# yamatokataoka/reinforcement-learning-replications

Hardware: AMD Instinct MI355X
Metric: env_steps_per_sec (higher is better)
Workload: dtype fp32; 1 GPU; model=PPO HalfCheetah-v4 (policy MLP [17,64,32,6] tanh, value [17,64,32,1]), global_batch=4000, seq_len=1000, parallelism=dp1, num_envs_per_gpu=200, env_residency=device, policy_grads_per_epoch=80

## Files before the change

rl_replicas_amd/algorithms/on_policy.py:

```python
from __future__ import annotations

import logging
from typing import Dict, List

import numpy as np
import torch
import torch.nn.functional as F
from torch import Tensor

from rl_replicas_amd import ops
from rl_replicas_amd.algorithms.base import AlgorithmBase
from rl_replicas_amd.experience import Experience
from rl_replicas_amd.policies import Policy
from rl_replicas_amd.samplers import Sampler
from rl_replicas_amd.value_function import ValueFunction

logger = logging.getLogger(__name__)


class OnPolicyAlgorithm(AlgorithmBase):
    def __init__(
        self,
        policy: Policy,
        value_function: ValueFunction,
        env,
        sampler: Sampler,
        gamma: float,
        gae_lambda: float,
        num_value_gradients: int,
    ) -> None:
        self.policy = policy
        self.value_function = value_function
        self.env = env
        self.sampler = sampler
        self.gamma = gamma
        self.gae_lambda = gae_lambda
        self.num_value_gradients = num_value_gradients

    def learn(
        self,
        num_epochs: int = 50,
        batch_size: int = 4000,
        model_saving_interval: int = 4000,
        output_dir: str = ".",
    ) -> None:
        import time as _time

        self._begin_learn(output_dir)
        for current_epoch in range(1, num_epochs + 1):
            t0 = _time.perf_counter()
            experience = self.sampler.sample(batch_size, self.policy)
            t1 = _time.perf_counter()

            self.current_total_steps += sum(experience.episode_lengths)
            self.current_total_episodes += sum(experience.episode_dones)

            self._record_sampling_metrics(
                current_epoch, experience.episode_returns, experience.episode_lengths
            )

            self.train(experience)

            self.metrics_manager.record_phase_ms("sample", (t1 - t0) * 1000.0)
            self.metrics_manager.record_phase_ms("train", (_time.perf_counter() - t1) * 1000.0)
            self.metrics_manager.dump_phases(self.current_total_steps)

            self._end_epoch(current_epoch, model_saving_interval, output_dir)
        self.metrics_manager.close()

    def _prepare_batch(self, experience: Experience) -> Dict[str, Tensor]:
        device = self.device
        flat = experience.to_flat_batch()
        if isinstance(flat["observations"], Tensor):
            obs = flat["observations"].to(device)
            actions = flat["actions"].to(device=device, dtype=torch.float32)
            rewards = flat["rewards"].to(device)
            last_obs = flat["last_observations"].to(device)
            return self._finish_batch(flat, obs, actions, rewards, last_obs, device)
        obs_np = flat["observations"]
        act_np = np.asarray(flat["actions"], dtype=np.float32)
        rew_np = flat["rewards"]
        last_np = flat["last_observations"]
        if device.type == "cuda":
            sizes = [a.size for a in (obs_np, act_np, rew_np, last_np)]
            total = int(sum(sizes))
            pinned = getattr(self, "_h2d_pinned", None)
            if pinned is None or pinned.numel() < total:
                pinned = torch.empty(total, dtype=torch.float32, pin_memory=True)
                self._h2d_pinned = pinned
                self._h2d_event = torch.cuda.Event()
            self._h2d_event.synchronize()
            host = pinned[:total].numpy()
            o = 0
            for a in (obs_np, act_np, rew_np, last_np):
                host[o : o + a.size] = a.reshape(-1)
                o += a.size
            dev_flat = pinned[:total].to(device, non_blocking=True)
            self._h2d_event.record()
            s0, s1, s2, s3 = np.cumsum(sizes)
            obs = dev_flat[:s0].view(obs_np.shape)
            actions = dev_flat[s0:s1].view(act_np.shape)
            rewards = dev_flat[s1:s2]
            last_obs = dev_flat[s2:s3].view(last_np.shape)
        else:
            obs = torch.as_tensor(obs_np, dtype=torch.float32, device=device)
            actions = torch.as_tensor(act_np, device=device)
            rewards = torch.as_tensor(rew_np, dtype=torch.float32, device=device)
            last_obs = torch.as_tensor(last_np, dtype=torch.float32, device=device)
        return self._finish_batch(flat, obs, actions, rewards, last_obs, device)

    def _finish_batch(self, flat, obs, actions, rewards, last_obs, device) -> Dict[str, Tensor]:
        offsets = torch.as_tensor(flat["episode_offsets"], device=device)
        dones = torch.as_tensor(flat["episode_dones"], device=device)

        with torch.no_grad():
            values_all = self.value_function(torch.cat([obs, last_obs], dim=0)).flatten()
        num_steps = obs.shape[0]
        values = values_all[:num_steps]
        last_values = values_all[num_steps:]

        advantages, returns = ops.gae_advantages_and_returns(
            rewards, values, last_values, offsets, dones, self.gamma, self.gae_lambda
        )
        obs, actions, advantages, returns = self._gather_global_batch(
            obs, actions, advantages, returns
        )
        advantages = self._normalize_advantages(advantages)
        return {
            "observations": obs,
            "actions": actions,
            "advantages": advantages.detach(),
            "discounted_returns": returns.detach(),
        }

    def _gather_global_batch(self, obs, actions, advantages, returns):
        return obs, actions, advantages, returns

    def _normalize_advantages(self, advantages: Tensor) -> Tensor:
        return ops.normalize(advantages)

    def train(self, experience: Experience) -> None:
        batch = self._prepare_batch(experience)
        obs = batch["observations"]
        actions = batch["actions"]
        advantages = batch["advantages"]
        returns = batch["discounted_returns"]

        joint = self._update_policy_and_value(obs, actions, advantages, returns)
        if joint is not None:
            policy_metrics, value_loss = joint
        else:
            policy_metrics = self._update_policy(obs, actions, advantages)
            value_loss = self._update_value_function(obs, returns)

        m = self.metrics_manager
        for tag, value in policy_metrics.items():
            m.record_scalar(tag, value, self.current_total_steps, tensorboard=True)
        m.record_scalar(
            "value_function/average_loss",
            value_loss,
            self.current_total_steps,
            tensorboard=True,
        )

    def _update_policy(self, obs: Tensor, actions: Tensor, advantages: Tensor) -> Dict[str, float]:
        raise NotImplementedError

    def _update_policy_and_value(self, obs: Tensor, actions: Tensor, advantages: Tensor,
                                 returns: Tensor):
        return None

    def _update_value_function(self, obs: Tensor, returns: Tensor) -> float:
        from rl_replicas_amd.ops import fused_onpolicy

        if fused_onpolicy.value_supported(self, obs):
            return fused_onpolicy.value_update(self, obs, returns, self.num_value_gradients)
        value_losses: List[float] = []
        for _ in range(self.num_value_gradients):
            value_losses.append(self.train_value_function(obs, returns).item())
        return float(np.mean(value_losses))

    def _policy_diagnostics(self, obs: Tensor, actions: Tensor) -> Dict[str, float]:
        with torch.no_grad():
            dist = self.policy(obs)
            log_probs = dist.log_prob(actions)
            entropies = dist.entropy()
        return {
            "policy/avarage_entropy": float(torch.mean(entropies)),
            "policy/log_prob_std": float(torch.std(log_probs)),
        }

    def train_value_function(self, observations: Tensor, discounted_returns: Tensor) -> Tensor:
        loss = self.compute_value_function_loss(observations, discounted_returns)
        self.value_function.optimizer.zero_grad()
        loss.backward()
        self._all_reduce_gradients(self.value_function)
        self.value_function.optimizer.step()
        return loss.detach()

    def compute_value_function_loss(self, observations: Tensor, discounted_returns: Tensor) -> Tensor:
        values = torch.squeeze(self.value_function(observations), -1)
        return F.mse_loss(values, discounted_returns)

    def _all_reduce_gradients(self, module) -> None:
        """DP hook: no-op single-process; the parallel wrapper overrides."""

    def _checkpoint_dict(self, epoch: int) -> Dict:
        return {
            "epoch": epoch,
            "total_steps": self.current_total_steps,
            "policy_state_dict": self.policy.network.state_dict(),
            "policy_optimizer_state_dict": self.policy.optimizer.state_dict(),
            "value_function_state_dict": self.value_function.network.state_dict(),
            "value_function_optimizer_state_dict": self.value_function.optimizer.state_dict(),
        }

    def _restore_from_checkpoint(self, ckpt: Dict) -> None:
        self.policy.network.load_state_dict(ckpt["policy_state_dict"])
        self.policy.optimizer.load_state_dict(ckpt["policy_optimizer_state_dict"])
        self.value_function.network.load_state_dict(ckpt["value_function_state_dict"])
        self.value_function.optimizer.load_state_dict(ckpt["value_function_optimizer_state_dict"])
```

rl_replicas_amd/algorithms/ppo.py:

```python
from __future__ import annotations

import copy
import logging
from typing import Dict

import torch
from torch import Tensor

from rl_replicas_amd.algorithms.on_policy import OnPolicyAlgorithm
from rl_replicas_amd.policies import Policy
from rl_replicas_amd.samplers import Sampler
from rl_replicas_amd.value_function import ValueFunction

logger = logging.getLogger(__name__)


class PPO(OnPolicyAlgorithm):
    def __init__(
        self,
        policy: Policy,
        value_function: ValueFunction,
        env,
        sampler: Sampler,
        gamma: float = 0.99,
        gae_lambda: float = 0.97,
        clip_range: float = 0.2,
        max_kl_divergence: float = 0.01,
        num_policy_gradients: int = 80,
        num_value_gradients: int = 80,
    ) -> None:
        super().__init__(policy, value_function, env, sampler, gamma, gae_lambda, num_value_gradients)
        self.clip_range = clip_range
        self.max_kl_divergence = max_kl_divergence
        self.num_policy_gradients = num_policy_gradients
        self.old_policy: Policy = copy.deepcopy(self.policy)

    def _update_policy(self, obs: Tensor, actions: Tensor, advantages: Tensor) -> Dict[str, float]:
        from rl_replicas_amd.ops import fused_onpolicy

        if fused_onpolicy.supported(self.policy, obs):
            return fused_onpolicy.ppo_update(self, obs, actions, advantages)
        diagnostics = self._policy_diagnostics(obs, actions)
        with torch.no_grad():
            loss_before = self.compute_policy_loss(obs, actions, advantages)

        with torch.no_grad():
            old_log_probs = self.old_policy(obs).log_prob(actions)

        approximate_kl = torch.zeros((), device=obs.device)
        for i in range(self.num_policy_gradients):
            self.train_policy(obs, actions, advantages, old_log_probs)
            with torch.no_grad():
                log_probs = self.policy(obs).log_prob(actions)
                approximate_kl = torch.mean(old_log_probs - log_probs)
            approximate_kl = self._reduce_scalar_mean(approximate_kl)
            if float(approximate_kl) > 1.5 * self.max_kl_divergence:
                logger.info(
                    "Early stopping at update %d due to reaching max KL divergence.", i
                )
                break

        self.old_policy.load_state_dict(self.policy.state_dict())

        return {
            "policy/loss": float(loss_before),
            **diagnostics,
            "policy/kl_divergence": float(approximate_kl),
        }

    def _update_policy_and_value(self, obs: Tensor, actions: Tensor, advantages: Tensor,
                                 returns: Tensor):
        from rl_replicas_amd.ops import fused_onpolicy

        if fused_onpolicy.ppo_twin_eligible(self, obs):
            return fused_onpolicy.ppo_value_twin_update(self, obs, actions, advantages, returns)
        return None

    def train_policy(self, obs: Tensor, actions: Tensor, advantages: Tensor, old_log_probs: Tensor) -> None:
        loss = self._clipped_loss(obs, actions, advantages, old_log_probs)
        self.policy.optimizer.zero_grad()
        loss.backward()
        self._all_reduce_gradients(self.policy)
        self.policy.optimizer.step()

    def _clipped_loss(self, obs: Tensor, actions: Tensor, advantages: Tensor, old_log_probs: Tensor) -> Tensor:
        log_probs = self.policy(obs).log_prob(actions)
        ratio = torch.exp(log_probs - old_log_probs)
        clipped_ratio = torch.clamp(ratio, 1.0 - self.clip_range, 1.0 + self.clip_range)
        return -torch.mean(torch.min(ratio * advantages, clipped_ratio * advantages))

    def compute_policy_loss(self, observations: Tensor, actions: Tensor, advantages: Tensor) -> Tensor:
        with torch.no_grad():
            old_log_probs = self.old_policy(observations).log_prob(actions)
        return self._clipped_loss(observations, actions, advantages, old_log_probs)

    def compute_approximate_kl_divergence(self, observations: Tensor, actions: Tensor) -> Tensor:
        with torch.no_grad():
            log_probs = self.policy(observations).log_prob(actions)
            old_log_probs = self.old_policy(observations).log_prob(actions)
        return torch.mean(old_log_probs - log_probs)
```

rl_replicas_amd/ops/fused_onpolicy.py:

```python
from __future__ import annotations

import gc
import logging
import math
import os
from typing import Dict, List, Optional

import numpy as np
import torch
from torch import Tensor

from rl_replicas_amd import ops
from rl_replicas_amd.ops.fused_mlp import _extract_layers
from rl_replicas_amd.policies import CategoricalPolicy, GaussianPolicy

logger = logging.getLogger(__name__)

MODE_VPG = 0
MODE_PPO = 1


def _policy_kind(policy) -> Optional[str]:
    if isinstance(policy, GaussianPolicy):
        return "gaussian"
# ... 356 lines not shown
                "policy/kl_divergence": float(self.kl_final[0]),
            }
        loss_before = None
        approximate_kl = 0.0
        for i in range(algo.num_policy_gradients):
            scalars = self.pre.replay()
            algo._all_reduce_gradients(policy)
            kl = self.post.replay()
            if loss_before is None:
                loss_before = float(scalars[0])
            approximate_kl = float(algo._reduce_scalar_mean(kl[0]))
            if approximate_kl > 1.5 * algo.max_kl_divergence:
                logger.info(
                    "Early stopping at update %d due to reaching max KL divergence.", i
                )
                break
        return {"policy/loss": loss_before, "policy/kl_divergence": approximate_kl}


def _value_iter_wide(algo, obs: Tensor, returns: Tensor, adam=None) -> Tensor:
    ext = ops._load_extension()
    vf = algo.value_function
    mlp = vf.network
    out, hidden, weights, biases, acts = _forward_saved(mlp, obs)
    dv, scalars = ext.value_mse_loss(out.view(-1), returns)
    if adam is not None:
        m, v, step0, hp, delta = adam
        ext.mlp_backward(dv.view(out.shape), obs, list(weights),
                         list(biases), list(hidden), out, acts,
                         ops.compute_bf16(), m, v, step0, *hp, delta)
        return scalars
    grads = ext.mlp_backward(dv.view(out.shape), obs, list(weights),
                             list(biases), list(hidden), out, acts,
                             ops.compute_bf16())
    _assign_grads(weights, biases, grads)
    return scalars


class _GraphedValueLoop:

    def __init__(self, algo, obs0: Tensor, returns0: Tensor, num_iters: int,
                 split: bool, mode: str = "narrow"):
        ext = ops._load_extension()
        vf = algo.value_function
        mlp = vf.network
        self.obs = obs0.clone()
        self.returns = returns0.clone()
        self.num_iters = num_iters
        self.split = split

        if mode == "wide":
            self._init_wide(algo, vf, num_iters, split)
            return

        def iter_pre():
            out, hidden, weights, biases, acts = _forward_saved(mlp, self.obs)
            grads = ext.value_mlp_backward(self.obs, list(weights), list(biases),
                                           list(hidden), out, acts, self.returns,
                                           ops.compute_bf16())
            _assign_grads(weights, biases, grads)
            return grads[-1]

        state = [p.data for p in vf.parameters()]
        state += _ensure_adam_state(vf.optimizer)
        if split:
            self.pre = _CapturedLoop(iter_pre, state)
            self.post = _CapturedLoop(lambda: vf.optimizer.step(), state)
        else:
            fb = int(ext.value_loss_partials_blocks(obs0.shape[0]))
            self.partials = torch.zeros(num_iters, fb, device=obs0.device)
            from rl_replicas_amd.ops.fused_adam import adam_arg_lists

            weights0, biases0, _ = _extract_layers(mlp)
            adam_m, adam_v, adam_step, hp = adam_arg_lists(
                vf.optimizer, weights0, biases0
            )

            fp32 = ops.compute_bf16() == 0 and _fwd_in_kernel_fits(weights0)
            dummy = torch.empty(0, device=obs0.device)

            def body():
                weights, biases, acts = _extract_layers(mlp)
                for i in range(num_iters):
                    if fp32:
                        ext.value_mlp_backward(
                            self.obs, list(weights), list(biases), [],
                            dummy, acts, self.returns, 0,
                            self.partials[i], adam_m, adam_v, adam_step,
                            *hp, float(i), True,
                        )
                    else:
                        out, hidden, _, _, _ = _forward_saved(mlp, self.obs)
                        ext.value_mlp_backward(
                            self.obs, list(weights), list(biases), list(hidden),
                            out, acts, self.returns, ops.compute_bf16(),
                            self.partials[i], adam_m, adam_v, adam_step,
                            *hp, float(i),
                        )
                vf.optimizer.bump_steps(float(num_iters))
                return ext.value_loss_finalize(self.partials, fb)

            self.loop = _CapturedLoop(body, state)

    def _init_wide(self, algo, vf, num_iters: int, split: bool) -> None:

        def iter_pre():
            return _value_iter_wide(algo, self.obs, self.returns)

        state = [p.data for p in vf.parameters()]
        state += _ensure_adam_state(vf.optimizer)
        if split:
            self.pre = _CapturedLoop(iter_pre, state)
            self.post = _CapturedLoop(lambda: vf.optimizer.step(), state)
        else:
            losses_buf = torch.zeros(num_iters, device=self.obs.device)
            from rl_replicas_amd.ops.fused_adam import adam_arg_lists

            weights0, biases0, _ = _extract_layers(vf.network)
            adam_m, adam_v, adam_step, hp = adam_arg_lists(
                vf.optimizer, weights0, biases0
            )

            def body():
                for i in range(num_iters):
                    losses_buf[i].copy_(
                        _value_iter_wide(
                            algo, self.obs, self.returns,
                            adam=(adam_m, adam_v, adam_step, hp, float(i)),
                        )[0]
                    )
                vf.optimizer.bump_steps(float(num_iters))
                return losses_buf

            self.loop = _CapturedLoop(body, state)

    def run(self, algo, obs, returns) -> float:
        self.obs.copy_(obs)
        self.returns.copy_(returns)
        if self.split:
            losses = []
            for _ in range(self.num_iters):
                losses.append(self.pre.replay().clone())
                algo._all_reduce_gradients(algo.value_function)
                self.post.replay()
            return float(torch.cat(losses).mean())
        losses = self.loop.replay()
        return float(losses.mean())


class _GraphedPPOTwin:

    def __init__(self, algo, obs0: Tensor, actions0: Tensor, adv0: Tensor,
                 old_logp0: Tensor, returns0: Tensor):
        from rl_replicas_amd.ops.fused_adam import adam_arg_lists

        ext = ops._load_extension()
        policy, vf = algo.policy, algo.value_function
        pmlp, vmlp = _mlp_of(policy), vf.network
        dev = obs0.device
        self.obs = obs0.clone()
        self.actions = actions0.clone()
        self.adv = adv0.clone()
        self.old_logp = old_logp0.clone()
        self.returns = returns0.clone()
        clip = float(algo.clip_range)
        thr = 1.5 * float(algo.max_kl_divergence)
        num_p = int(algo.num_policy_gradients)
        num_v = int(algo.num_value_gradients)
        assert 1 <= num_p <= num_v
        self.gate = torch.ones(1, device=dev)
        self.kl_final = torch.zeros(1, device=dev)
        self.loss0 = torch.zeros(1, device=dev)
        self.iters_done = torch.zeros(1, device=dev)
        scratch_loss = torch.zeros(1, device=dev)

        pw, pb, pacts = _extract_layers(pmlp)
        pm, pv, pstep, php = adam_arg_lists(policy.optimizer, pw, pb)
        state = [p.data for p in policy.parameters()]
        state += _ensure_adam_state(policy.optimizer)
        kind = _policy_kind(policy)
        self.kind = kind
        twin_iter, seed_args, ls_mv = _policy_iter_binding(
            ext, policy, kind, twin=True
        )

        vw, vb, vacts = _extract_layers(vmlp)
        vm, vv, vstep, vhp = adam_arg_lists(vf.optimizer, vw, vb)
        state += [p.data for p in vf.parameters()]
        state += _ensure_adam_state(vf.optimizer)
        fb = int(ext.value_loss_partials_blocks(obs0.shape[0]))
        self.partials = torch.zeros(num_v, fb, device=dev)
        dummy = torch.empty(0, device=dev)

        def body():
            self.gate.fill_(1.0)
            self.iters_done.zero_()
            for i in range(num_p):
                twin_iter(
                    self.obs, list(pw), list(pb), pacts, self.actions,
                    self.old_logp, self.adv, *seed_args, clip, pm,
                    pv, *ls_mv, pstep, *php, float(i), self.gate,
                    self.kl_final, self.iters_done, thr,
                    self.loss0 if i == 0 else scratch_loss, i == 0,
                    self.obs, list(vw), list(vb), vacts, self.returns,
                    self.partials[i], vm, vv, vstep, *vhp, float(i),
                )
            for i in range(num_p, num_v):
                ext.value_mlp_backward(
                    self.obs, list(vw), list(vb), [], dummy, vacts,
                    self.returns, 0, self.partials[i], vm, vv, vstep, *vhp,
                    float(i), True,
                )
            out = _forward_only(pmlp, self.obs)
            if kind == "gaussian":
                kl = ext.gaussian_kl(out, self.actions, policy.log_std.data,
                                     self.old_logp)
            else:
                kl = ext.categorical_kl(out, self.actions, self.old_logp)
            ext.ppo_gate_update_(self.gate, kl, self.kl_final,
                                 self.iters_done, thr)
            policy.optimizer.bump_steps_by(self.iters_done)
            vf.optimizer.bump_steps(float(num_v))
            return ext.value_loss_finalize(self.partials, fb)

        self.loop = _CapturedLoop(body, state)

    def run(self, algo, obs, actions, advantages, old_logp, returns):
        self.obs.copy_(obs)
        self.actions.copy_(actions.view(self.actions.shape))
        self.adv.copy_(advantages)
        self.old_logp.copy_(old_logp)
        self.returns.copy_(returns)
        losses = self.loop.replay()
        iters = int(self.iters_done)
        if iters < algo.num_policy_gradients:
            logger.info(
                "Early stopping at update %d due to reaching max KL divergence.",
                iters - 1,
            )
        return {
            "policy/loss": float(self.loss0[0]),
            "policy/kl_divergence": float(self.kl_final[0]),
        }, float(losses.mean())


def _get_cached_graph(algo, attr: str, key, builder):
    cached = getattr(algo, attr, None)
    if cached is not None and cached[0] == key:
        return cached[1]
    graph = builder()
    setattr(algo, attr, (key, graph))
    return graph


def _kernel_inputs(policy, obs: Tensor, actions: Tensor, advantages: Tensor):
    kind = _policy_kind(policy)
    obs = obs.contiguous()
    if kind == "gaussian":
        actions_k = actions.contiguous().view(obs.shape[0], -1)
    else:
        actions_k = actions.contiguous().view(-1)
    advantages = advantages.contiguous()
    diagnostics = _fast_diagnostics(policy, kind, obs, actions_k)
    return kind, obs, actions_k, advantages, diagnostics


def _ppo_prelude(algo, obs: Tensor, actions: Tensor, advantages: Tensor):
    kind, obs, actions_k, advantages, diagnostics = _kernel_inputs(
        algo.policy, obs, actions, advantages
    )
    with torch.no_grad():
        old_logp = _old_logp(algo.old_policy, kind, obs, actions_k)
    return kind, obs, actions_k, advantages, diagnostics, old_logp


def ppo_twin_eligible(algo, obs: Tensor) -> bool:
    if os.environ.get("RL_REPLICAS_AMD_PPO_TWIN", "1") == "0":
        return False
    policy = algo.policy
    if not supported(policy, obs) or value_mode(algo, obs) != "narrow":
        return False
    if not 1 <= int(algo.num_policy_gradients) <= int(algo.num_value_gradients):
        return False
    if not (_graphs_enabled(algo) and _graphs_enabled_value(algo)) or _dp_active(algo):
        return False
    if not _mega_eligible(policy, _policy_kind(policy), obs):
        return False
    vweights = _extract_layers(algo.value_function.network)[0]
    if not _fwd_in_kernel_fits(vweights):
        return False
    ext = ops._load_extension()
    fb = int(ext.value_loss_partials_blocks(obs.shape[0]))
    pweights = _extract_layers(_mlp_of(policy))[0]
    grand_p = sum(w.numel() + w.shape[0] for w in pweights)
    if _policy_kind(policy) == "gaussian":
        grand_p += policy.log_std.numel()
    grand_v = sum(w.numel() + w.shape[0] for w in vweights)
    return bool(ext.reduce_adam_is_staged(fb, grand_p)
                and ext.reduce_adam_is_staged(fb, grand_v))


def ppo_value_twin_update(algo, obs: Tensor, actions: Tensor, advantages: Tensor,
                          returns: Tensor):
    policy = algo.policy
    kind, obs, actions_k, advantages, diagnostics, old_logp = _ppo_prelude(
        algo, obs, actions, advantages
    )
    returns = returns.contiguous()
    key = (tuple(obs.shape), tuple(actions_k.shape),
           int(algo.num_policy_gradients), int(algo.num_value_gradients),
           tuple(id(p) for p in policy.parameters()),
           tuple(id(p) for p in algo.value_function.parameters()))
    graphed = _get_cached_graph(
        algo, "_ppo_twin_graph", key,
        lambda: _GraphedPPOTwin(algo, obs, actions_k, advantages, old_logp, returns),
    )
    metrics, value_loss = graphed.run(algo, obs, actions_k, advantages, old_logp,
                                      returns)
    algo.old_policy.load_state_dict(policy.state_dict())
    return {
        "policy/loss": metrics["policy/loss"],
        **diagnostics,
        "policy/kl_divergence": metrics["policy/kl_divergence"],
    }, value_loss


def ppo_update(algo, obs: Tensor, actions: Tensor, advantages: Tensor) -> Dict[str, float]:
    ext = ops._load_extension()
    policy = algo.policy
    mlp = _mlp_of(policy)
    kind, obs, actions_k, advantages, diagnostics, old_logp = _ppo_prelude(
        algo, obs, actions, advantages
    )

    if _graphs_enabled(algo):
        split = _dp_active(algo)
        key = (kind, tuple(obs.shape), tuple(actions_k.shape), split,
               tuple(id(p) for p in policy.parameters()))
        graphed = _get_cached_graph(
            algo, "_ppo_policy_graph", key,
            lambda: _GraphedPPO(algo, kind, obs, actions_k, advantages, old_logp, split),
        )
        metrics = graphed.run(algo, obs, actions_k, advantages, old_logp)
        algo.old_policy.load_state_dict(policy.state_dict())
        return {
            "policy/loss": metrics["policy/loss"],
            **diagnostics,
            "policy/kl_divergence": metrics["policy/kl_divergence"],
        }

    clip = float(algo.clip_range)
    loss_before: Optional[Tensor] = None
    approximate_kl = torch.zeros((), device=obs.device)
    for i in range(algo.num_policy_gradients):
        out, hidden, weights, biases, acts = _forward_saved(mlp, obs)
        grad_out, extra, scalars = _policy_loss(
            policy, kind, MODE_PPO, out, actions_k, old_logp, advantages, clip
        )
        if loss_before is None:
            loss_before = scalars[0]
        _backward_and_step(
            policy, mlp, obs, grad_out, hidden, out, weights, biases, acts,
            extra, algo._all_reduce_gradients,
        )
        new_out = _forward_only(mlp, obs)
        if kind == "gaussian":
            kl = ext.gaussian_kl(new_out, actions_k, policy.log_std.data, old_logp)
        else:
            kl = ext.categorical_kl(new_out, actions_k, old_logp)
        approximate_kl = algo._reduce_scalar_mean(kl[0])
        if float(approximate_kl) > 1.5 * algo.max_kl_divergence:
            logger.info("Early stopping at update %d due to reaching max KL divergence.", i)
            break

    algo.old_policy.load_state_dict(policy.state_dict())
    return {
        "policy/loss": float(loss_before),
        **diagnostics,
        "policy/kl_divergence": float(approximate_kl),
    }


def vpg_update(algo, obs: Tensor, actions: Tensor, advantages: Tensor) -> Dict[str, float]:
    policy = algo.policy
    mlp = _mlp_of(policy)
    kind, obs, actions_k, advantages, diagnostics = _kernel_inputs(
        policy, obs, actions, advantages
    )

    out, hidden, weights, biases, acts = _forward_saved(mlp, obs)
    dummy = torch.empty(0, device=obs.device)
    grad_out, extra, scalars = _policy_loss(
        policy, kind, MODE_VPG, out, actions_k, dummy, advantages, 0.0
    )
    _backward_and_step(
        policy, mlp, obs, grad_out, hidden, out, weights, biases, acts, extra,
# ... 60 lines not shown
```

rl_replicas_amd/ops/hip/bindings.hip:

```cpp
#include <torch/extension.h>

#include <c10/hip/HIPStream.h>
#include <hip/hip_runtime.h>

#include <vector>

#include "common.h"

void launch_mlp_fwd(const MLPArgs& args, const float* x, int save_hidden,
                    int rows, int n_blocks, size_t lds_bytes, int compute_bf16,
                    hipStream_t stream);
void launch_mlp_bwd_layer(const float* dy, const float* y, const float* xin,
                          const float* W, float* dx, float* ws, long ws_stride,
                          int batch, int out_d, int in_d, int act, int rows,
                          int n_blocks, size_t lds_bytes, hipStream_t stream);
void launch_mlp_bwd_fused(const MLPBwdArgs& args, const float* x,
                          const float* dy, float* dx, float* ws,
                          const float* mse_returns, float* loss_partials,
                          size_t lds_bytes, int n_blocks, int compute_bf16,
                          hipStream_t stream, int do_fwd = 0,
                          GaussSeedArgs gargs = GaussSeedArgs{},
                          int need_dx = 1);
__global__ void mlp_grad_reduce_onepass_f32(ReduceAllArgs a);
void launch_mlp_grad_reduce_adam(const ReduceAdamArgs& a, long grand,
                                 hipStream_t stream);
void launch_mlp_bwd_fused_twin(const MLPBwdTwinArgs& a, size_t lds_bytes,
                               int n_blocks, hipStream_t stream);
void launch_mlp_bwd_fused_twin_shaped(const MLPBwdTwinArgs& a, int n_blocks,
                                      hipStream_t stream);
size_t mlp_bwd_fused_shaped_lds(int in_d);
bool mlp_reduce_adam_is_staged(int n_blocks, long grand);
void launch_mlp_grad_reduce_adam_twin(const ReduceAdamArgs& pol, long grand_pol,
                                      const ReduceAdamArgs& val, long grand_val,
                                      hipStream_t stream);
void launch_mlp_layer_fwd_wide(const float* x, const float* W, const float* B,
                               float* out, int batch, int in_d, int out_d,
                               int act, hipStream_t stream);
void launch_mlp_bwd_wide(const float* dy, const float* y, const float* xin,
                         const float* W, float* dx, float* ws, long ws_stride,
                         int batch, int out_d, int in_d, int act,
                         hipStream_t stream);
void launch_mlp_dgrad_wide(const float* dy, const float* y, const float* W,
                           float* dx, int batch, int out_d, int in_d, int act,
                           hipStream_t stream);
void launch_gaussian_loss(const float* mean, const float* actions,
                          const float* old_logp, const float* adv,
                          const float* log_std, float* dmean, float* c_buf,
                          float* partials, int B, int D, float clip, int mode,
                          int n_blocks, hipStream_t stream);
__global__ void loss_partials_finalize(const float* partials, float* dlog_std,
                                       float* scalars, int n_blocks, int D);
__global__ void gaussian_logp_kernel(const float* mean, const float* actions,
                                     const float* log_std, float* logp, int B,
                                     int D);
__global__ void gaussian_kl_kernel(const float* mean, const float* actions,
                                   const float* log_std, const float* old_logp,
                                   float* out, int B, int D);
__global__ void categorical_policy_loss_bwd(const float* logits,
                                            const float* actions,
                                            const float* old_logp,
                                            const float* adv, float* dlogits,
                                            float* partials, int B, int N,
                                            float clip, int mode);
__global__ void categorical_logp_kernel(const float* logits, const float* actions,
                                        float* logp, int B, int N);
__global__ void categorical_kl_kernel(const float* logits, const float* actions,
                                      const float* old_logp, float* out, int B,
                                      int N);
__global__ void value_loss_finalize_rows(const float* partials, float* scalars,
                                         int rows, int fb, int row_stride);
__global__ void value_mse_bwd_kernel(const float* v, const float* ret, float* dv,
                                     float* scalars, int B);
__global__ void gaussian_sample_kernel(const float* mean, const float* log_std,
                                       float* out, int B, int D, uint64_t seed,
                                       uint64_t offset, float noise_scale,
                                       float limit,
                                       const unsigned long long* offset_ptr);
__global__ void categorical_sample_kernel(const float* logits, int64_t* out,
                                          int B, int N, uint64_t seed,
                                          uint64_t offset,
                                          const unsigned long long* offset_ptr);
__global__ void cartpole_env_step_kernel(double* state, int* elapsed,
                                         const int64_t* actions, float* obs,
                                         float* final_obs, float* reward,
                                         uint8_t* done, int N, int max_steps,
                                         uint64_t seed, uint64_t offset,
                                         const unsigned long long* offset_ptr);
__global__ void cartpole_env_reset_kernel(double* state, int* elapsed, float* obs,
                                          int N, uint64_t seed, uint64_t offset,
                                          const unsigned long long* offset_ptr);
void launch_cartpole_rollout_fused(const CartPoleRolloutArgs& a, hipStream_t stream);
__global__ void pendulum_env_step_kernel(double* state, const float* actions,
                                         float* obs, float* final_obs,
                                         float* reward, int N, int do_reset,
                                         uint64_t seed, uint64_t offset,
                                         const unsigned long long* offset_ptr);
__global__ void pendulum_env_reset_kernel(double* state, float* obs, int N,
                                          int draw, uint64_t seed, uint64_t offset,
                                          const unsigned long long* offset_ptr);
void launch_pendulum_rollout_fused(const PendulumRolloutArgs& a, hipStream_t stream);
void launch_pendulum_collect_fused(const PendulumCollectArgs& a, int wide_threads,
                                   hipStream_t stream);
void launch_pendulum_eval_fused(const PendulumEvalArgs& a, int wide_threads,
                                hipStream_t stream);
void launch_cartpole_eval_fused(const CartPoleEvalArgs& a, hipStream_t stream);
__global__ void episode_reduce_kernel(const float* rew_buf,
                                      const unsigned char* done_buf, double* returns,
                                      int* lengths, int N, int steps);
__global__ void uniform_sample_kernel(float* out, int total, float low, float high,
                                      uint64_t seed, uint64_t offset,
                                      const unsigned long long* offset_ptr);
__global__ void replay_scatter_kernel(ReplayScatterArgs a);
__global__ void ring_advance_kernel(long long* write, long long* size,
                                    unsigned long long n, unsigned long long cap);
__global__ void synthetic_env_step_kernel(const float* state, const float* actions,
                                          const float* A, const float* Bm,
                                          const float* w, float* s_out,
                                          float* final_out, float* reward, int N,
                                          int O, int Adim, float sigma,
                                          uint64_t seed, uint64_t offset,
                                          int do_reset,
                                          const unsigned long long* offset_ptr);
__global__ void synthetic_env_reset_kernel(float* s_out, int total,
                                           uint64_t seed, uint64_t offset,
                                           const unsigned long long* offset_ptr);
__global__ void counter_add_kernel(unsigned long long* ctr,
                                   unsigned long long delta);
void launch_ppo_rollout_fused(const RolloutFusedArgs& a, hipStream_t stream);
__global__ void segmented_gae_kernel(const float* rewards, const float* values,
                                     const float* last_values, const int* offsets,
                                     const int* dones, float* advantages,
                                     float* returns, float gamma, float lam);
__global__ void normalize_kernel(const float* x, float* y, int n);
__global__ void q_target_kernel(const float* r, const float* d, const float* qn,
                                float* out, float gamma, int n);
__global__ void td3_smooth_kernel(const float* a, float* out, int total,
                                  uint64_t seed, uint64_t offset, float scale,
                                  float clip, float limit,
                                  const unsigned long long* offset_ptr);
__global__ void q_target_min2_kernel(const float* r, const float* d,
                                     const float* q1, const float* q2,
                                     float* out, float gamma, int n);
__global__ void replay_gather_kernel(ReplayGatherArgs a);

__global__ void fused_adam_kernel(AdamArgs a);
__global__ void adam_step_bump_kernel(AdamArgs a);
__global__ void fused_polyak_kernel(PolyakArgs a);
__global__ void ppo_gate_update_kernel(float* gate, const float* kl,
                                       float* kl_final, float* iters_done,
                                       float thr);

namespace {

hipStream_t current_stream() { return c10::hip::getCurrentHIPStream().stream(); }

void check_f32_gpu(const torch::Tensor& t, const char* name) {
  TORCH_CHECK(t.is_cuda(), name, " must be on GPU");
  TORCH_CHECK(t.scalar_type() == torch::kFloat32, name, " must be fp32");
  TORCH_CHECK(t.is_contiguous(), name, " must be contiguous");
}

#define HIP_OK(expr)                                                        \
  do {                                                                      \
    hipError_t _e = (expr);                                                 \
    TORCH_CHECK(_e == hipSuccess, "HIP error: ", hipGetErrorString(_e));    \
  } while (0)

constexpr int BWD_FUSED_ROWS = 32;

struct NetLayout {
  int L = 0;
  int dims[MLP_MAX_LAYERS + 1] = {};
  int64_t totals[MLP_MAX_LAYERS] = {};
  int64_t layer_off[MLP_MAX_LAYERS] = {};
  int64_t grand = 0;
  size_t whole_w = 0;
  int max_width = 0;
};

NetLayout net_layout(const std::vector<int64_t>& dims, int width_cap,
                     int reserve = 0) {
  NetLayout n;
  n.L = (int)dims.size() - 1;
  TORCH_CHECK(n.L >= 1 && n.L + reserve <= MLP_MAX_LAYERS,
              "unsupported layer count ", n.L, " (at most ",
              MLP_MAX_LAYERS - reserve, ")");
  for (int l = 0; l <= n.L; ++l) {
    TORCH_CHECK(dims[l] >= 1 && dims[l] <= width_cap, "layer width ", dims[l],
                " outside [1, ", width_cap, "]");
    n.dims[l] = (int)dims[l];
    n.max_width = std::max(n.max_width, n.dims[l]);
  }
  for (int l = 0; l < n.L; ++l) {
    n.totals[l] = (int64_t)n.dims[l + 1] * n.dims[l] + n.dims[l + 1];
    n.layer_off[l] = n.grand;
    n.grand += n.totals[l];
    n.whole_w += (size_t)n.dims[l + 1] * (n.dims[l] + 1);
  }
  return n;
}

NetLayout net_layout(int64_t in_dim, const std::vector<torch::Tensor>& weights,
                     const std::vector<torch::Tensor>& biases,
                     const std::vector<int64_t>& acts, int width_cap,
                     int reserve = 0) {
  TORCH_CHECK(biases.size() == weights.size() && acts.size() == weights.size(),
              "weights/biases/acts length mismatch");
  std::vector<int64_t> dims{in_dim};
  for (size_t l = 0; l < weights.size(); ++l) {
    check_f32_gpu(weights[l], "weight");
    check_f32_gpu(biases[l], "bias");
    TORCH_CHECK(weights[l].dim() == 2 && weights[l].size(1) == dims[l],
                "weight shape mismatch at layer ", l);
    TORCH_CHECK(biases[l].numel() == weights[l].size(0),
                "bias shape mismatch at layer ", l);
    dims.push_back(weights[l].size(0));
  }
  return net_layout(dims, width_cap, reserve);
}

NetLayout net_layout(const torch::Tensor& x,
                     const std::vector<torch::Tensor>& weights,
                     const std::vector<torch::Tensor>& biases,
                     const std::vector<int64_t>& acts, int width_cap,
                     int reserve = 0) {
  check_f32_gpu(x, "x");
  TORCH_CHECK(x.dim() == 2, "x must be 2-D");
  return net_layout(x.size(1), weights, biases, acts, width_cap, reserve);
}

template <class Args>
void fill_net(Args& a, const NetLayout& n,
              const std::vector<torch::Tensor>& weights,
              const std::vector<torch::Tensor>& biases,
              const std::vector<int64_t>& acts) {
  a.n_layers = n.L;
  a.dims[0] = n.dims[0];
  for (int l = 0; l < n.L; ++l) {
    a.w[l] = weights[l].data_ptr<float>();
    a.b[l] = biases[l].data_ptr<float>();
    a.dims[l + 1] = n.dims[l + 1];
    a.acts[l] = (int)acts[l];
  }
}

void check_saved(const NetLayout& n, int64_t batch,
                 const std::vector<torch::Tensor>& hidden,
                 const torch::Tensor& final_out) {
  TORCH_CHECK((int)hidden.size() == n.L - 1, "hidden must hold ", n.L - 1,
              " activations, got ", hidden.size());
  for (int l = 0; l < n.L; ++l) {
    const torch::Tensor& h = l == n.L - 1 ? final_out : hidden[l];
    check_f32_gpu(h, "saved activation");
    TORCH_CHECK(h.numel() == batch * n.dims[l + 1],
                "saved activation shape mismatch at layer ", l);
  }
}

void check_adam_state(const std::vector<torch::Tensor>& weights,
                      const std::vector<torch::Tensor>& biases,
                      const std::vector<torch::Tensor>& m,
                      const std::vector<torch::Tensor>& v,
                      const torch::Tensor& step) {
  const size_t L = weights.size();
  TORCH_CHECK(m.size() == 2 * L && v.size() == 2 * L,
              "adam m/v must be [weights..., biases...] (2L tensors)");
  for (size_t i = 0; i < 2 * L; ++i) {
    const torch::Tensor& p = i < L ? weights[i] : biases[i - L];
    check_f32_gpu(m[i], "adam m");
    check_f32_gpu(v[i], "adam v");
    TORCH_CHECK(m[i].numel() == p.numel() && v[i].numel() == p.numel(),
                "adam state shape mismatch");
  }
  TORCH_CHECK(step.is_cuda() && step.scalar_type() == torch::kFloat32 &&
                  step.numel() == 1,
              "adam step must be a 1-element fp32 GPU tensor");
}

size_t two_tile_lds(int rows, size_t image_floats) {
  return ((size_t)2 * rows * (MLP_NARROW_WIDTH + 4) + image_floats) * 4;
}
// ... 355 lines not shown
                     mean.data_ptr<float>(), actions.data_ptr<float>(),
                     log_std.data_ptr<float>(), old_logp.data_ptr<float>(),
                     out.data_ptr<float>(), B, D);
  HIP_OK(hipGetLastError());
  return out;
}

std::vector<torch::Tensor> categorical_policy_loss(torch::Tensor logits,
                                                   torch::Tensor actions,
                                                   torch::Tensor old_logp,
                                                   torch::Tensor adv, double clip,
                                                   int64_t mode) {
  check_f32_gpu(logits, "logits");
  const int B = (int)logits.size(0);
  const int N = (int)logits.size(1);
  auto dlogits = torch::empty_like(logits);
  auto scalars = torch::empty({1}, logits.options());
  const int n_blocks = std::min(32, (B + 255) / 256);
  auto partials = torch::empty({n_blocks}, logits.options());
  const float* olp = mode == 1 ? old_logp.data_ptr<float>() : nullptr;
  auto stream = current_stream();
  hipLaunchKernelGGL(categorical_policy_loss_bwd, dim3(n_blocks), dim3(256), 0,
                     stream, logits.data_ptr<float>(),
                     actions.data_ptr<float>(), olp, adv.data_ptr<float>(),
                     dlogits.data_ptr<float>(), partials.data_ptr<float>(), B, N,
                     (float)clip, (int)mode);
  HIP_OK(hipGetLastError());
  hipLaunchKernelGGL(loss_partials_finalize, dim3(1), dim3(1), 0, stream,
                     partials.data_ptr<float>(), nullptr,
                     scalars.data_ptr<float>(), n_blocks, 0);
  HIP_OK(hipGetLastError());
  return {dlogits, scalars};
}

torch::Tensor categorical_logp(torch::Tensor logits, torch::Tensor actions) {
  check_f32_gpu(logits, "logits");
  const int B = (int)logits.size(0);
  const int N = (int)logits.size(1);
  auto logp = torch::empty({B}, logits.options());
  hipLaunchKernelGGL(categorical_logp_kernel, dim3(std::min(64, (B + 1023) / 1024)),
                     dim3(1024), 0, current_stream(), logits.data_ptr<float>(),
                     actions.data_ptr<float>(), logp.data_ptr<float>(), B, N);
  HIP_OK(hipGetLastError());
  return logp;
}

torch::Tensor categorical_kl(torch::Tensor logits, torch::Tensor actions,
                             torch::Tensor old_logp) {
  check_f32_gpu(logits, "logits");
  const int B = (int)logits.size(0);
  const int N = (int)logits.size(1);
  auto out = torch::empty({1}, logits.options());
  hipLaunchKernelGGL(categorical_kl_kernel, dim3(1), dim3(1024), 0,
                     current_stream(), logits.data_ptr<float>(),
                     actions.data_ptr<float>(), old_logp.data_ptr<float>(),
                     out.data_ptr<float>(), B, N);
  HIP_OK(hipGetLastError());
  return out;
}

std::vector<torch::Tensor> value_mse_loss(torch::Tensor v, torch::Tensor ret) {
  check_f32_gpu(v, "v");
  const int B = (int)v.numel();
  auto dv = torch::empty_like(v);
  auto scalars = torch::empty({1}, v.options());
  hipLaunchKernelGGL(value_mse_bwd_kernel, dim3(1), dim3(1024), 0,
                     current_stream(), v.data_ptr<float>(), ret.data_ptr<float>(),
                     dv.data_ptr<float>(), scalars.data_ptr<float>(), B);
  HIP_OK(hipGetLastError());
  return {dv, scalars};
}

std::vector<torch::Tensor> value_mlp_backward(torch::Tensor x,
                                              std::vector<torch::Tensor> weights,
                                              std::vector<torch::Tensor> biases,
                                              std::vector<torch::Tensor> hidden,
                                              torch::Tensor final_out,
                                              std::vector<int64_t> acts,
                                              torch::Tensor returns,
                                              int64_t compute_bf16,
                                              c10::optional<torch::Tensor> partials_out,
                                              c10::optional<std::vector<torch::Tensor>> adam_m,
                                              c10::optional<std::vector<torch::Tensor>> adam_v,
                                              c10::optional<torch::Tensor> adam_step,
                                              double lr, double beta1,
                                              double beta2, double eps,
                                              double weight_decay,
                                              double adam_step_delta,
                                              bool fwd_in_kernel) {
  const bool fuse_adam = adam_m.has_value();
  TORCH_CHECK(!fwd_in_kernel || compute_bf16 == 0,
              "fwd_in_kernel is fp32-only");
  const NetLayout net = net_layout(x, weights, biases, acts, MLP_NARROW_WIDTH);
  const int L = net.L;
  const int batch = (int)x.size(0);
  check_f32_gpu(returns, "returns");
  TORCH_CHECK(returns.numel() == batch, "returns must be [batch]");
  TORCH_CHECK(net.dims[L] == 1 && acts[L - 1] == 0,
              "value_mlp_backward needs a 1-output identity head");
  TORCH_CHECK(fused_bwd_fits(net, fwd_in_kernel),
              "net too large for fused value backward");
  if (!fwd_in_kernel) check_saved(net, batch, hidden, final_out);
  if (fuse_adam) {
    TORCH_CHECK(adam_v.has_value() && adam_step.has_value(),
                "adam_m needs adam_v and adam_step");
    check_adam_state(weights, biases, *adam_m, *adam_v, *adam_step);
  }
  const int fb = (batch + BWD_FUSED_ROWS - 1) / BWD_FUSED_ROWS;
  const bool deferred = partials_out.has_value();
  if (deferred) {
    check_f32_gpu(*partials_out, "partials_out");
    TORCH_CHECK(partials_out->numel() >= fb, "partials_out too small");
  }
  auto opts = x.options();
  auto stream = current_stream();

  const int64_t grand = net.grand;
  torch::Tensor ws = torch::empty({(int64_t)fb, grand}, opts);
  torch::Tensor loss_partials = deferred ? *partials_out : torch::empty({fb}, opts);
  torch::Tensor scalars = torch::empty({1}, opts);
  const GradOut g(net, opts);
  MLPBwdArgs ba = fill_bwd_args(x, weights, biases, acts, net, grand);
  if (!fwd_in_kernel) set_saved(ba, net, hidden, final_out);
  torch::Tensor dx = fuse_adam ? torch::empty({0}, opts)
                               : torch::empty({batch, x.size(1)}, opts);
  launch_mlp_bwd_fused(ba, x.data_ptr<float>(), nullptr,
                       fuse_adam ? nullptr : dx.data_ptr<float>(),
                       ws.data_ptr<float>(), returns.data_ptr<float>(),
                       loss_partials.data_ptr<float>(),
                       fused_bwd_lds(net, fwd_in_kernel), fb,
                       (int)compute_bf16, stream, fwd_in_kernel ? 1 : 0,
                       GaussSeedArgs{}, fuse_adam ? 0 : 1);
  HIP_OK(hipGetLastError());

  if (fuse_adam) {
    launch_reduce_adam(weights, biases, net, ws.data_ptr<float>(), fb,
                       *adam_m, *adam_v, *adam_step, lr, beta1, beta2, eps,
                       weight_decay, adam_step_delta, c10::nullopt, stream);
  } else {
    launch_reduce_all(net, ws.data_ptr<float>(), fb, g, stream);
  }
  if (!deferred) {
    hipLaunchKernelGGL(loss_partials_finalize, dim3(1), dim3(1), 0, stream,
                       loss_partials.data_ptr<float>(), nullptr,
                       scalars.data_ptr<float>(), fb, 0);
    HIP_OK(hipGetLastError());
  }

  std::vector<torch::Tensor> out = g.pack(dx);
  out.push_back(scalars);
  return out;
}

std::vector<torch::Tensor> segmented_gae(torch::Tensor rewards, torch::Tensor values,
                                         torch::Tensor last_values,
                                         torch::Tensor offsets, torch::Tensor dones,
                                         double gamma, double lam) {
  check_f32_gpu(rewards, "rewards");
  check_f32_gpu(values, "values");
  check_f32_gpu(last_values, "last_values");
  TORCH_CHECK(offsets.scalar_type() == torch::kInt32 && offsets.is_cuda());
  TORCH_CHECK(dones.scalar_type() == torch::kInt32 && dones.is_cuda());
  const int n_eps = (int)last_values.size(0);
  auto adv = torch::empty_like(rewards);
  auto ret = torch::empty_like(rewards);
  if (n_eps > 0) {
    hipLaunchKernelGGL(segmented_gae_kernel, dim3(n_eps), dim3(256), 0,
                       current_stream(), rewards.data_ptr<float>(),
                       values.data_ptr<float>(), last_values.data_ptr<float>(),
                       offsets.data_ptr<int>(), dones.data_ptr<int>(),
                       adv.data_ptr<float>(), ret.data_ptr<float>(), (float)gamma,
                       (float)lam);
    HIP_OK(hipGetLastError());
  }
  return {adv, ret};
}

torch::Tensor normalize(torch::Tensor x) {
  check_f32_gpu(x, "x");
  auto y = torch::empty_like(x);
  hipLaunchKernelGGL(normalize_kernel, dim3(1), dim3(1024), 0, current_stream(),
                     x.data_ptr<float>(), y.data_ptr<float>(), (int)x.numel());
  HIP_OK(hipGetLastError());
  return y;
}

torch::Tensor q_target(torch::Tensor r, torch::Tensor d, torch::Tensor qn,
                       double gamma) {
  check_f32_gpu(r, "rewards");
  auto out = torch::empty_like(r);
  int n = (int)r.numel();
  hipLaunchKernelGGL(q_target_kernel, dim3((n + 255) / 256), dim3(256), 0,
                     current_stream(), r.data_ptr<float>(), d.data_ptr<float>(),
                     qn.data_ptr<float>(), out.data_ptr<float>(), (float)gamma, n);
  HIP_OK(hipGetLastError());
  return out;
}

void fused_adam_(std::vector<torch::Tensor> params, std::vector<torch::Tensor> grads,
                 std::vector<torch::Tensor> exp_avgs,
                 std::vector<torch::Tensor> exp_avg_sqs,
                 std::vector<torch::Tensor> steps, double lr, double beta1,
                 double beta2, double eps, double weight_decay,
                 double step_delta, bool do_bump,
                 c10::optional<torch::Tensor> gate) {
  const float* gate_ptr = nullptr;
  if (gate.has_value()) {
    TORCH_CHECK(gate->scalar_type() == torch::kFloat32 && gate->is_cuda() &&
                    gate->numel() == 1,
                "gate must be a 1-element fp32 CUDA tensor");
    gate_ptr = gate->data_ptr<float>();
  }
  size_t n = params.size();
  for (size_t base = 0; base < n; base += MT_MAX_TENSORS) {
    AdamArgs a{};
    a.n_tensors = (int)std::min((size_t)MT_MAX_TENSORS, n - base);
    for (int i = 0; i < a.n_tensors; ++i) {
      size_t t = base + i;
      a.p[i] = params[t].data_ptr<float>();
      a.g[i] = grads[t].data_ptr<float>();
      a.m[i] = exp_avgs[t].data_ptr<float>();
      a.v[i] = exp_avg_sqs[t].data_ptr<float>();
      a.step[i] = steps[t].data_ptr<float>();
      a.numel[i] = (int)params[t].numel();
    }
    a.lr = (float)lr;
    a.beta1 = (float)beta1;
    a.beta2 = (float)beta2;
    a.eps = (float)eps;
    a.weight_decay = (float)weight_decay;
    a.step_delta = (float)step_delta;
    a.gate = gate_ptr;
    int max_chunks = 1;
    for (int i = 0; i < a.n_tensors; ++i)
      max_chunks = std::max(max_chunks, (a.numel[i] + 8191) / 8192);
    hipLaunchKernelGGL(fused_adam_kernel, dim3(a.n_tensors, max_chunks),
                       dim3(256), 0, current_stream(), a);
    HIP_OK(hipGetLastError());
    if (do_bump) {
      a.step_delta = 1.f;
      hipLaunchKernelGGL(adam_step_bump_kernel, dim3(1), dim3(MT_MAX_TENSORS), 0,
                         current_stream(), a);
      HIP_OK(hipGetLastError());
    }
  }
}

__global__ void adam_step_bump_dev_kernel(AdamArgs a, const float* amount);

void adam_bump_dev_(std::vector<torch::Tensor> steps, torch::Tensor amount) {
  size_t n = steps.size();
  for (size_t base = 0; base < n; base += MT_MAX_TENSORS) {
    AdamArgs a{};
    a.n_tensors = (int)std::min((size_t)MT_MAX_TENSORS, n - base);
    for (int i = 0; i < a.n_tensors; ++i)
      a.step[i] = steps[base + i].data_ptr<float>();
    hipLaunchKernelGGL(adam_step_bump_dev_kernel, dim3(1), dim3(MT_MAX_TENSORS),
                       0, current_stream(), a, amount.data_ptr<float>());
    HIP_OK(hipGetLastError());
  }
}

void adam_bump_(std::vector<torch::Tensor> steps, double amount) {
  size_t n = steps.size();
  for (size_t base = 0; base < n; base += MT_MAX_TENSORS) {
    AdamArgs a{};
    a.n_tensors = (int)std::min((size_t)MT_MAX_TENSORS, n - base);
    for (int i = 0; i < a.n_tensors; ++i)
      a.step[i] = steps[base + i].data_ptr<float>();
    a.step_delta = (float)amount;
    hipLaunchKernelGGL(adam_step_bump_kernel, dim3(1), dim3(MT_MAX_TENSORS), 0,
                       current_stream(), a);
    HIP_OK(hipGetLastError());
  }
}

torch::Tensor value_loss_finalize(torch::Tensor partials, int64_t fb) {
  check_f32_gpu(partials, "partials");
  const int rows = (int)partials.size(0);
  const int stride = (int)partials.size(1);
  TORCH_CHECK((int)fb <= stride, "fb exceeds partials row stride");
  auto scalars = torch::empty({rows}, partials.options());
  hipLaunchKernelGGL(value_loss_finalize_rows, dim3((rows + 3) / 4),
                     dim3(256), 0, current_stream(),
                     partials.data_ptr<float>(), scalars.data_ptr<float>(),
                     rows, (int)fb, stride);
  HIP_OK(hipGetLastError());
  return scalars;
}

void fused_polyak_(std::vector<torch::Tensor> srcs, std::vector<torch::Tensor> dsts,
                   double rho) {
  size_t n = srcs.size();
  for (size_t base = 0; base < n; base += MT_MAX_TENSORS) {
    PolyakArgs a{};
    a.n_tensors = (int)std::min((size_t)MT_MAX_TENSORS, n - base);
    for (int i = 0; i < a.n_tensors; ++i) {
      size_t t = base + i;
      a.src[i] = srcs[t].data_ptr<float>();
      a.dst[i] = dsts[t].data_ptr<float>();
      a.numel[i] = (int)srcs[t].numel();
    }
    a.rho = (float)rho;
    int max_chunks = 1;
    for (int i = 0; i < a.n_tensors; ++i)
      max_chunks = std::max(max_chunks, (a.numel[i] + 8191) / 8192);
    hipLaunchKernelGGL(fused_polyak_kernel, dim3(a.n_tensors, max_chunks),
                       dim3(256), 0, current_stream(), a);
    HIP_OK(hipGetLastError());
  }
}

static const unsigned long long* ctr_ptr(const c10::optional<torch::Tensor>& t) {
  if (!t.has_value()) return nullptr;
  TORCH_CHECK(t->scalar_type() == torch::kInt64 && t->is_cuda() && t->numel() == 1,
              "offset_ctr must be a 1-element int64 CUDA tensor");
  return reinterpret_cast<const unsigned long long*>(t->data_ptr<int64_t>());
}

torch::Tensor gaussian_sample(torch::Tensor mean, torch::Tensor log_std,
                              int64_t seed, int64_t offset, double noise_scale,
                              double limit,
                              c10::optional<torch::Tensor> offset_ctr,
                              c10::optional<torch::Tensor> out_opt) {
  check_f32_gpu(mean, "mean");
  const int B = (int)mean.size(0);
  const int D = (int)mean.size(1);
  auto out = out_opt.has_value() ? *out_opt : torch::empty_like(mean);
  const int total = B * D;
  hipLaunchKernelGGL(gaussian_sample_kernel,
                     dim3(std::min(256, (total + 255) / 256)), dim3(256), 0,
                     current_stream(), mean.data_ptr<float>(),
                     log_std.data_ptr<float>(), out.data_ptr<float>(), B, D,
                     (uint64_t)seed, (uint64_t)offset, (float)noise_scale,
                     (float)limit, ctr_ptr(offset_ctr));
  HIP_OK(hipGetLastError());
  return out;
}

torch::Tensor categorical_sample(torch::Tensor logits, int64_t seed,
                                 int64_t offset,
                                 c10::optional<torch::Tensor> offset_ctr,
                                 c10::optional<torch::Tensor> out_opt) {
  check_f32_gpu(logits, "logits");
  const int B = (int)logits.size(0);
  const int N = (int)logits.size(1);
  auto out = out_opt.has_value()
                 ? *out_opt
                 : torch::empty({B}, logits.options().dtype(torch::kInt64));
  TORCH_CHECK(out.is_cuda() && out.is_contiguous() &&
                  out.scalar_type() == torch::kInt64 && out.numel() == B,
              "categorical_sample: out must be a contiguous int64 CUDA tensor [B]");
  hipLaunchKernelGGL(categorical_sample_kernel,
                     dim3(std::min(256, (B + 255) / 256)), dim3(256), 0,
                     current_stream(), logits.data_ptr<float>(),
                     out.data_ptr<int64_t>(), B, N, (uint64_t)seed,
                     (uint64_t)offset, ctr_ptr(offset_ctr));
  HIP_OK(hipGetLastError());
  return out;
}

static int check_cartpole_carry(const torch::Tensor& state,
                                const torch::Tensor& elapsed) {
  TORCH_CHECK(state.is_cuda() && state.is_contiguous() &&
                  state.scalar_type() == torch::kFloat64 && state.dim() == 2 &&
                  state.size(1) == 4,
              "state must be a contiguous float64 CUDA tensor [N, 4]");
  TORCH_CHECK(elapsed.is_cuda() && elapsed.is_contiguous() &&
                  elapsed.scalar_type() == torch::kInt32 &&
                  elapsed.numel() == state.size(0),
              "elapsed must be a contiguous int32 CUDA tensor [N]");
  return (int)state.size(0);
}

static void check_out(const torch::Tensor& t, torch::ScalarType dt, int64_t numel,
                      const char* name) {
  TORCH_CHECK(t.is_cuda() && t.is_contiguous() && t.scalar_type() == dt &&
                  t.numel() == numel,
              name, ": wrong device, dtype, layout or size");
}

#define DEFAULT_LDS_LIMIT (64 * 1024)

static size_t persistent_lds_bytes(const NetLayout& n) {
  return (size_t)net_lds_floats(3, n.dims, n.L) * sizeof(float);
}

static size_t ppo_rollout_fused_lds_bytes(const NetLayout& n, int O, int A) {
  return (size_t)rollout_fused_lds_floats(n.dims, n.L, O, A) * sizeof(float);
}

static int check_step_count(int64_t v, const char* name) {
  TORCH_CHECK(v >= 1 && v <= (1 << 24), name, " out of range");
  return (int)v;
}

static void check_net_device(const std::vector<torch::Tensor>& weights,
                             const std::vector<torch::Tensor>& biases,
                             const torch::Device& dev) {
  for (const auto& t : weights)
    TORCH_CHECK(t.device() == dev, "the net is on another device");
  for (const auto& t : biases)
    TORCH_CHECK(t.device() == dev, "the net is on another device");
}

template <class Args>
static void fill_cuts(Args& a, const std::vector<int64_t>& cuts, int64_t steps,
                      const char* who) {
  TORCH_CHECK(cuts.size() <= ROLLOUT_MAX_CUTS, who, ": too many cuts");
  a.n_cuts = (int)cuts.size();
  for (int c = 0; c < a.n_cuts; ++c) {
    TORCH_CHECK(cuts[c] >= 0 && cuts[c] < steps, "cut step out of range");
    TORCH_CHECK(c == 0 || cuts[c] > cuts[c - 1], "cuts must be ascending");
    a.cut_step[c] = (int)cuts[c];
  }
}

std::vector<torch::Tensor> cartpole_env_step(
    torch::Tensor state, torch::Tensor elapsed, torch::Tensor actions,
    int64_t max_steps, int64_t seed, int64_t offset,
    c10::optional<torch::Tensor> offset_ctr, c10::optional<torch::Tensor> obs_opt,
    c10::optional<torch::Tensor> final_opt, c10::optional<torch::Tensor> reward_opt,
    c10::optional<torch::Tensor> done_opt) {
  const int N = check_cartpole_carry(state, elapsed);
  check_out(actions, torch::kInt64, N, "actions");
  const auto f32 = state.options().dtype(torch::kFloat32);
  auto obs = obs_opt.has_value() ? *obs_opt : torch::empty({N, 4}, f32);
  auto fin = final_opt.has_value() ? *final_opt : torch::empty({N, 4}, f32);
  auto reward = reward_opt.has_value() ? *reward_opt : torch::empty({N}, f32);
  auto done = done_opt.has_value()
                  ? *done_opt
                  : torch::empty({N}, state.options().dtype(torch::kUInt8));
  check_out(obs, torch::kFloat32, (int64_t)N * 4, "obs");
  check_out(fin, torch::kFloat32, (int64_t)N * 4, "final_obs");
  check_out(reward, torch::kFloat32, N, "reward");
  check_out(done, torch::kUInt8, N, "done");
  hipLaunchKernelGGL(cartpole_env_step_kernel,
                     dim3(std::min(256, (N + 255) / 256)), dim3(256), 0,
                     current_stream(), state.data_ptr<double>(),
                     elapsed.data_ptr<int>(), actions.data_ptr<int64_t>(),
                     obs.data_ptr<float>(), fin.data_ptr<float>(),
// ... 673 lines not shown
  HIP_OK(hipGetLastError());
}

int64_t pendulum_rollout_fused_lds_bytes_py(std::vector<int64_t> dims) {
  const NetLayout n = net_layout(dims, ROLLOUT_MAX_WIDTH);
  return (int64_t)persistent_lds_bytes(n);
}

void pendulum_rollout_fused(std::vector<torch::Tensor> weights,
                            std::vector<torch::Tensor> biases,
                            std::vector<int64_t> acts, torch::Tensor log_std,
                            int64_t policy_seed, int64_t env_seed,
                            std::vector<int64_t> cuts, bool start_with_reset,
                            torch::Tensor ctr, torch::Tensor state,
                            torch::Tensor obs_full, torch::Tensor act_buf,
                            torch::Tensor rew_buf, torch::Tensor cut_final) {
  const NetLayout net = net_layout(3, weights, biases, acts, ROLLOUT_MAX_WIDTH);
  const int L = net.L;
  PendulumRolloutArgs a{};
  a.N = check_pendulum_carry(state);
  TORCH_CHECK(net.dims[L] == 1, "pendulum_rollout_fused: the policy head must be 1 wide");
  check_f32_gpu(log_std, "log_std");
  TORCH_CHECK(log_std.numel() == 1, "pendulum_rollout_fused: log_std must have 1 element");
  check_f32_gpu(obs_full, "obs_full");
  TORCH_CHECK(obs_full.dim() == 3 && obs_full.size(0) >= 2 &&
                  obs_full.size(1) == a.N && obs_full.size(2) == 3,
              "obs_full must be [steps+1, N, 3]");
  a.steps = (int)obs_full.size(0) - 1;
  const int64_t SN = (int64_t)a.steps * a.N;
  check_out(act_buf, torch::kFloat32, SN, "act_buf");
  check_out(rew_buf, torch::kFloat32, SN, "rew_buf");
  fill_cuts(a, cuts, a.steps, "pendulum_rollout_fused");
  check_f32_gpu(cut_final, "cut_final");
  TORCH_CHECK(cut_final.dim() == 3 && cut_final.size(0) >= std::max(a.n_cuts, 1) &&
                  cut_final.size(1) == a.N && cut_final.size(2) == 3,
              "cut_final must be [n_cuts, N, 3]");
  fill_net(a, net, weights, biases, acts);
  TORCH_CHECK(persistent_lds_bytes(net) <= DEFAULT_LDS_LIMIT,
              "pendulum_rollout_fused: net image exceeds the LDS budget");
  a.ctr = ctr_ptr(c10::optional<torch::Tensor>(ctr));
  a.log_std = log_std.data_ptr<float>();
  a.state = state.data_ptr<double>();
  a.obs_full = obs_full.data_ptr<float>();
  a.act_buf = act_buf.data_ptr<float>();
  a.rew_buf = rew_buf.data_ptr<float>();
  a.cut_final = cut_final.data_ptr<float>();
  a.start_with_reset = start_with_reset ? 1 : 0;
  a.policy_seed = (uint64_t)policy_seed;
  a.env_seed = (uint64_t)env_seed;
  launch_pendulum_rollout_fused(a, current_stream());
  HIP_OK(hipGetLastError());
}

static ReplayRing check_ring(const std::vector<torch::Tensor>& storage,
                             const torch::Tensor& write_dev,
                             const torch::Tensor& size_dev, int64_t n,
                             const torch::Device& dev) {
  TORCH_CHECK(storage.size() == 5,
              "ring storage must be [obs, act, rew, next_obs, dones]");
  static const char* names[5] = {"ring observations", "ring actions", "ring rewards",
                                 "ring next_observations", "ring dones"};
  for (int i = 0; i < 5; ++i) {
    check_f32_gpu(storage[i], names[i]);
    TORCH_CHECK(storage[i].device() == dev, names[i], " is on another device");
    TORCH_CHECK(storage[i].dim() >= 1, names[i], " must have a slot dimension");
  }
  const int64_t cap = storage[2].numel();
  TORCH_CHECK(cap >= 1, "empty ring");
  const int64_t per_slot[5] = {3, 1, 1, 3, 1};
  for (int i = 0; i < 5; ++i)
    TORCH_CHECK(storage[i].size(0) == cap && storage[i].numel() == cap * per_slot[i],
                names[i], " must hold ", per_slot[i], " floats per ring slot");
  for (const torch::Tensor* s : {&write_dev, &size_dev})
    TORCH_CHECK(s->scalar_type() == torch::kInt64 && s->is_cuda() &&
                    s->numel() == 1 && s->device() == dev,
                "ring scalars must be 1-element int64 tensors on the ring's device");
  TORCH_CHECK(n >= 1 && n <= cap, "an epoch of ", n,
              " transitions does not fit a ring of ", cap);
  ReplayRing r{};
  r.obs = storage[0].data_ptr<float>();
  r.act = storage[1].data_ptr<float>();
  r.rew = storage[2].data_ptr<float>();
  r.nxt = storage[3].data_ptr<float>();
  r.dn = storage[4].data_ptr<float>();
  r.write = reinterpret_cast<const long long*>(write_dev.data_ptr<int64_t>());
  r.cap = (unsigned long long)cap;
  return r;
}

static int epoch_segments(const std::vector<int64_t>& cuts, int64_t steps) {
  return (int)cuts.size() + ((cuts.empty() || cuts.back() != steps - 1) ? 1 : 0);
}

int64_t pendulum_collect_fused_lds_bytes_py(std::vector<int64_t> dims) {
  const NetLayout n = net_layout(dims, MLP_MAX_WIDTH);
  return (int64_t)persistent_lds_bytes(n);
}

void pendulum_collect_fused(std::vector<torch::Tensor> weights,
                            std::vector<torch::Tensor> biases,
                            std::vector<int64_t> acts, int64_t mode,
                            double noise_scale, double limit, double low,
                            double high, int64_t action_seed, int64_t env_seed,
                            std::vector<int64_t> cuts, bool start_with_reset,
                            torch::Tensor ctr, torch::Tensor state, int64_t steps,
                            std::vector<torch::Tensor> storage,
                            torch::Tensor write_dev, torch::Tensor size_dev,
                            torch::Tensor seg_returns, torch::Tensor last_obs,
                            int64_t wide_threads) {
  PendulumCollectArgs a{};
  a.N = check_pendulum_carry(state);
  a.steps = check_step_count(steps, "steps");
  a.ring = check_ring(storage, write_dev, size_dev, (int64_t)a.N * steps,
                      state.device());
  TORCH_CHECK(mode == COLLECT_NOISED || mode == COLLECT_UNIFORM, "unknown mode");
  a.mode = (int)mode;
  NetLayout net;
  if (mode == COLLECT_NOISED) {
    net = net_layout(3, weights, biases, acts, MLP_MAX_WIDTH);
    TORCH_CHECK(net.dims[net.L] == 1,
                "pendulum_collect_fused: the actor head must be 1 wide");
    check_net_device(weights, biases, state.device());
    TORCH_CHECK(noise_scale >= 0.0 && limit >= 0.0,
                "pendulum_collect_fused: noise_scale and limit must be >= 0");
    fill_net(a, net, weights, biases, acts);
  } else {
    TORCH_CHECK(weights.empty() && biases.empty() && acts.empty(),
                "pendulum_collect_fused: uniform mode takes no net");
    TORCH_CHECK(low <= high, "pendulum_collect_fused: low > high");
  }
  TORCH_CHECK(persistent_lds_bytes(net) <= MLP_LDS_BUDGET,
              "pendulum_collect_fused: net image exceeds the LDS budget");
  TORCH_CHECK(wide_threads == 256 || wide_threads == 1024,
              "pendulum_collect_fused: wide_threads must be 256 or 1024");
  fill_cuts(a, cuts, steps, "pendulum_collect_fused");
  a.n_segs = epoch_segments(cuts, steps);
  check_out(seg_returns, torch::kFloat32, (int64_t)a.N * a.n_segs, "seg_returns");
  check_out(last_obs, torch::kFloat32, (int64_t)a.N * 3, "last_obs");
  TORCH_CHECK(seg_returns.device() == state.device() &&
                  last_obs.device() == state.device(),
              "seg_returns / last_obs are on another device");
  a.ctr = ctr_ptr(c10::optional<torch::Tensor>(ctr));
  a.state = state.data_ptr<double>();
  a.seg_returns = seg_returns.data_ptr<float>();
  a.last_obs = last_obs.data_ptr<float>();
  a.start_with_reset = start_with_reset ? 1 : 0;
  a.noise_scale = (float)noise_scale;
  a.limit = (float)limit;
  a.low = (float)low;
  a.high = (float)high;
  a.action_seed = (uint64_t)action_seed;
  a.env_seed = (uint64_t)env_seed;
  launch_pendulum_collect_fused(a, (int)wide_threads, current_stream());
  HIP_OK(hipGetLastError());
}

static int check_eval_outputs(const torch::Tensor& returns,
                              const torch::Tensor& lengths,
                              const torch::Tensor& init_state, int state_dim) {
  TORCH_CHECK(returns.is_cuda() && returns.is_contiguous() &&
                  returns.scalar_type() == torch::kFloat64 && returns.dim() == 1 &&
                  returns.size(0) >= 1,
              "returns must be a contiguous float64 CUDA tensor [N]");
  const int64_t N = returns.size(0);
  TORCH_CHECK(N < (1LL << 24), "too many episodes");
  TORCH_CHECK(lengths.is_cuda() && lengths.is_contiguous() &&
                  lengths.scalar_type() == torch::kInt32 && lengths.dim() == 1 &&
                  lengths.size(0) == N,
              "lengths must be a contiguous int32 CUDA tensor [N]");
  TORCH_CHECK(init_state.is_cuda() && init_state.is_contiguous() &&
                  init_state.scalar_type() == torch::kFloat64 &&
                  init_state.dim() == 2 && init_state.size(0) == N &&
                  init_state.size(1) == state_dim,
              "init_state must be a contiguous float64 CUDA tensor [N, ", state_dim, "]");
  TORCH_CHECK(lengths.device() == returns.device() &&
                  init_state.device() == returns.device(),
              "returns / lengths / init_state are on different devices");
  return (int)N;
}

static void check_eval_counters(const torch::Tensor& ctr, const torch::Tensor& reset_ctr,
                                const torch::Device& dev) {
  for (const torch::Tensor* c : {&ctr, &reset_ctr})
    TORCH_CHECK(c->scalar_type() == torch::kInt64 && c->is_cuda() && c->numel() == 1 &&
                    c->device() == dev,
                "ctr / reset_ctr must be 1-element int64 tensors on the outputs' device");
}

int64_t pendulum_eval_fused_lds_bytes_py(std::vector<int64_t> dims) {
  const NetLayout n = net_layout(dims, MLP_MAX_WIDTH);
  return (int64_t)persistent_lds_bytes(n);
}

int64_t cartpole_eval_fused_lds_bytes_py(std::vector<int64_t> dims) {
  const NetLayout n = net_layout(dims, ROLLOUT_MAX_WIDTH);
  return (int64_t)persistent_lds_bytes(n);
}

void pendulum_eval_fused(std::vector<torch::Tensor> weights,
                         std::vector<torch::Tensor> biases,
                         std::vector<int64_t> acts, int64_t mode,
                         c10::optional<torch::Tensor> log_std, int64_t policy_seed,
                         int64_t env_seed, int64_t horizon, torch::Tensor ctr,
                         torch::Tensor reset_ctr, torch::Tensor returns,
                         torch::Tensor lengths, torch::Tensor init_state,
                         int64_t wide_threads) {
  PendulumEvalArgs a{};
  a.N = check_eval_outputs(returns, lengths, init_state, 2);
  check_eval_counters(ctr, reset_ctr, returns.device());
  a.horizon = check_step_count(horizon, "horizon");
  TORCH_CHECK(mode == EVAL_DETERMINISTIC || mode == EVAL_GAUSSIAN, "unknown mode");
  a.mode = (int)mode;
  const NetLayout net = net_layout(3, weights, biases, acts, MLP_MAX_WIDTH);
  TORCH_CHECK(net.dims[net.L] == 1, "pendulum_eval_fused: the policy head must be 1 wide");
  check_net_device(weights, biases, returns.device());
  if (mode == EVAL_GAUSSIAN) {
    TORCH_CHECK(log_std.has_value(), "pendulum_eval_fused: Gaussian mode needs log_std");
    check_f32_gpu(*log_std, "log_std");
    TORCH_CHECK(log_std->numel() == 1 && log_std->device() == returns.device(),
                "pendulum_eval_fused: log_std must have 1 element on the outputs' device");
    a.log_std = log_std->data_ptr<float>();
  }
  fill_net(a, net, weights, biases, acts);
  TORCH_CHECK(persistent_lds_bytes(net) <= DEFAULT_LDS_LIMIT,
              "pendulum_eval_fused: net image exceeds the LDS budget");
  TORCH_CHECK(wide_threads == 256 || wide_threads == 1024,
              "pendulum_eval_fused: wide_threads must be 256 or 1024");
  a.returns = returns.data_ptr<double>();
  a.lengths = lengths.data_ptr<int>();
  a.init_state = init_state.data_ptr<double>();
  a.ctr = ctr_ptr(c10::optional<torch::Tensor>(ctr));
  a.reset_ctr = ctr_ptr(c10::optional<torch::Tensor>(reset_ctr));
  a.policy_seed = (uint64_t)policy_seed;
  a.env_seed = (uint64_t)env_seed;
  launch_pendulum_eval_fused(a, (int)wide_threads, current_stream());
  HIP_OK(hipGetLastError());
}

void cartpole_eval_fused(std::vector<torch::Tensor> weights,
                         std::vector<torch::Tensor> biases,
                         std::vector<int64_t> acts, int64_t policy_seed,
                         int64_t env_seed, int64_t horizon, torch::Tensor ctr,
                         torch::Tensor reset_ctr, torch::Tensor returns,
                         torch::Tensor lengths, torch::Tensor init_state) {
  CartPoleEvalArgs a{};
  a.N = check_eval_outputs(returns, lengths, init_state, 4);
  check_eval_counters(ctr, reset_ctr, returns.device());
  a.horizon = check_step_count(horizon, "horizon");
  const NetLayout net = net_layout(4, weights, biases, acts, ROLLOUT_MAX_WIDTH);
  check_net_device(weights, biases, returns.device());
  fill_net(a, net, weights, biases, acts);
  TORCH_CHECK(persistent_lds_bytes(net) <= DEFAULT_LDS_LIMIT,
              "cartpole_eval_fused: net image exceeds the LDS budget");
  a.returns = returns.data_ptr<double>();
  a.lengths = lengths.data_ptr<int>();
  a.init_state = init_state.data_ptr<double>();
  a.ctr = ctr_ptr(c10::optional<torch::Tensor>(ctr));
  a.reset_ctr = ctr_ptr(c10::optional<torch::Tensor>(reset_ctr));
  a.policy_seed = (uint64_t)policy_seed;
  a.env_seed = (uint64_t)env_seed;
  launch_cartpole_eval_fused(a, current_stream());
  HIP_OK(hipGetLastError());
}

void episode_reduce(torch::Tensor rew_buf, c10::optional<torch::Tensor> done_buf,
                    torch::Tensor returns, torch::Tensor lengths) {
  check_f32_gpu(rew_buf, "rew_buf");
  TORCH_CHECK(rew_buf.dim() == 2 && rew_buf.size(0) >= 1 && rew_buf.size(1) >= 1 &&
                  rew_buf.size(0) <= (1 << 24) && rew_buf.size(1) < (1 << 24),
              "rew_buf must be [steps, N]");
  const int steps = (int)rew_buf.size(0);
  const int N = (int)rew_buf.size(1);
  const unsigned char* dn = nullptr;
  if (done_buf.has_value()) {
    check_out(*done_buf, torch::kUInt8, (int64_t)steps * N, "done_buf");
    TORCH_CHECK(done_buf->device() == rew_buf.device(), "episode_reduce: mixed devices");
    dn = done_buf->data_ptr<uint8_t>();
  }
  check_out(returns, torch::kFloat64, N, "returns");
  check_out(lengths, torch::kInt32, N, "lengths");
  TORCH_CHECK(returns.device() == rew_buf.device() && lengths.device() == rew_buf.device(),
              "episode_reduce: mixed devices");
  hipLaunchKernelGGL(episode_reduce_kernel, dim3(std::min(256, (N + 255) / 256)),
                     dim3(256), 0, current_stream(), rew_buf.data_ptr<float>(), dn,
                     returns.data_ptr<double>(), lengths.data_ptr<int>(), N, steps);
  HIP_OK(hipGetLastError());
}

void uniform_sample(torch::Tensor out, double low, double high, int64_t seed,
                    int64_t offset, c10::optional<torch::Tensor> offset_ctr) {
  check_f32_gpu(out, "out");
  TORCH_CHECK(low <= high, "uniform_sample: low > high");
  TORCH_CHECK(out.numel() < (1LL << 31), "uniform_sample: out too large");
  const int total = (int)out.numel();
  if (total == 0) return;
  hipLaunchKernelGGL(uniform_sample_kernel,
                     dim3(std::min(256, (total + 255) / 256)), dim3(256), 0,
                     current_stream(), out.data_ptr<float>(), total, (float)low,
                     (float)high, (uint64_t)seed, (uint64_t)offset,
                     ctr_ptr(offset_ctr));
  HIP_OK(hipGetLastError());
}

void replay_scatter(torch::Tensor obs_full, torch::Tensor act_buf,
                    torch::Tensor rew_buf, torch::Tensor cut_final,
                    torch::Tensor cut_slot, int64_t n_cuts,
// ... 105 lines not shown
        py::arg("offset_ctr") = py::none());
  m.def("replay_scatter", &replay_scatter,
        "ring write of one captured Pendulum epoch's buffers (gfx950)",
        py::arg("obs_full"), py::arg("act_buf"), py::arg("rew_buf"),
        py::arg("cut_final"), py::arg("cut_slot"), py::arg("n_cuts"),
        py::arg("storage"), py::arg("write_dev"), py::arg("size_dev"),
        py::arg("seg_returns"));
  m.def("ring_advance_", &ring_advance_,
        "advance the replay ring's device write position and fill (gfx950)");
  m.def("pendulum_rollout_fused", &pendulum_rollout_fused,
        "whole-epoch Pendulum rollout in one persistent kernel (gfx950)",
        py::arg("weights"), py::arg("biases"), py::arg("acts"),
        py::arg("log_std"), py::arg("policy_seed"), py::arg("env_seed"),
        py::arg("cuts"), py::arg("start_with_reset"), py::arg("ctr"),
        py::arg("state"), py::arg("obs_full"), py::arg("act_buf"),
        py::arg("rew_buf"), py::arg("cut_final"));
  m.def("pendulum_rollout_fused_lds_bytes", &pendulum_rollout_fused_lds_bytes_py,
        "dynamic LDS of pendulum_rollout_fused for a net [3, ..., 1]");
  m.def("pendulum_rollout_fused_limits",
        []() {
          return std::vector<int64_t>{MLP_MAX_LAYERS, ROLLOUT_MAX_WIDTH,
                                      ROLLOUT_MAX_CUTS, DEFAULT_LDS_LIMIT};
        },
        "(max layers, max width, max cuts, LDS budget in bytes) of "
        "pendulum_rollout_fused");
  m.def("pendulum_env_step", &pendulum_env_step,
        "Pendulum transition + lockstep autoreset (gfx950)", py::arg("state"),
        py::arg("actions"), py::arg("do_reset"), py::arg("seed"),
        py::arg("offset"), py::arg("offset_ctr") = py::none(),
        py::arg("obs") = py::none(), py::arg("final_obs") = py::none(),
        py::arg("reward") = py::none());
  m.def("pendulum_env_reset", &pendulum_env_reset,
        "Pendulum init states, or (draw=False) the observation of `state`",
        py::arg("state"), py::arg("seed"), py::arg("offset"),
        py::arg("offset_ctr") = py::none(), py::arg("obs") = py::none(),
        py::arg("draw") = true);
  m.def("cartpole_rollout_fused", &cartpole_rollout_fused,
        "whole-epoch CartPole rollout in one persistent kernel (gfx950)",
        py::arg("weights"), py::arg("biases"), py::arg("acts"),
        py::arg("policy_seed"), py::arg("env_seed"), py::arg("max_steps"),
        py::arg("start_with_reset"), py::arg("ctr"), py::arg("state"),
        py::arg("elapsed"), py::arg("obs_full"), py::arg("final_obs"),
        py::arg("act_buf"), py::arg("rew_buf"), py::arg("done_buf"));
  m.def("cartpole_rollout_fused_lds_bytes", &cartpole_rollout_fused_lds_bytes_py,
        "dynamic LDS of cartpole_rollout_fused for a net [4, ..., n_act]");
  m.def("cartpole_rollout_fused_limits",
        []() {
          return std::vector<int64_t>{MLP_MAX_LAYERS, ROLLOUT_MAX_WIDTH,
                                      DEFAULT_LDS_LIMIT};
        },
        "(max layers, max width, LDS budget in bytes) of cartpole_rollout_fused");
  m.def("cartpole_env_step", &cartpole_env_step,
        "CartPole transition + termination + autoreset (gfx950)",
        py::arg("state"), py::arg("elapsed"), py::arg("actions"),
        py::arg("max_steps"), py::arg("seed"), py::arg("offset"),
        py::arg("offset_ctr") = py::none(), py::arg("obs") = py::none(),
        py::arg("final_obs") = py::none(), py::arg("reward") = py::none(),
        py::arg("done") = py::none());
  m.def("cartpole_env_reset", &cartpole_env_reset,
        "CartPole init states (gfx950)", py::arg("state"), py::arg("elapsed"),
        py::arg("seed"), py::arg("offset"), py::arg("offset_ctr") = py::none(),
        py::arg("obs") = py::none());
  m.def("ppo_rollout_fused", &ppo_rollout_fused,
        "whole-epoch PPO rollout in one persistent kernel (gfx950)",
        py::arg("weights"), py::arg("biases"), py::arg("acts"),
        py::arg("log_std"), py::arg("env_A"), py::arg("env_B"), py::arg("env_w"),
        py::arg("sigma"), py::arg("policy_seed"), py::arg("env_seed"),
        py::arg("cuts"), py::arg("start_with_reset"), py::arg("ctr"),
        py::arg("obs_full"), py::arg("act_buf"), py::arg("rew_buf"),
        py::arg("cut_final"));
  m.def("ppo_rollout_fused_lds_bytes", &ppo_rollout_fused_lds_bytes_py,
        "dynamic LDS of ppo_rollout_fused for a net [O, ..., A]");
  m.def("ppo_rollout_fused_limits",
        []() {
          return std::vector<int64_t>{MLP_MAX_LAYERS, ROLLOUT_MAX_WIDTH,
                                      ROLLOUT_MAX_CUTS, (int64_t)MLP_LDS_BUDGET};
        },
        "(max layers, max width / obs dim, max cuts, LDS budget in bytes) of "
        "ppo_rollout_fused");
  m.def("fused_mlp_limits",
        []() {
          return std::vector<int64_t>{MLP_MAX_LAYERS, MLP_MAX_WIDTH,
                                      MLP_NARROW_WIDTH, GAUSS_MAX_D};
        },
        "(max layers, max width, max width of the whole-net LDS-image "
        "kernels = max action dim of the fused policy iteration, max action "
        "dim of the Gaussian loss kernel)");
  m.def("fused_bwd_fits",
        [](std::vector<int64_t> dims, int64_t reserve) {
          try {
            const NetLayout n = net_layout(dims, MLP_MAX_WIDTH, (int)reserve);
            return std::vector<bool>{fused_bwd_fits(n, false),
                                     fused_bwd_fits(n, true)};
          } catch (const c10::Error&) {
            return std::vector<bool>{false, false};
          }
        },
        "whether the whole-net fused backward takes a net [in, ..., out]: "
        "(with a separate forward, with the forward in the kernel); reserve "
        "= argument-block slots kept free (1 for the log_std pseudo-layer)",
        py::arg("dims"), py::arg("reserve") = 0);
  m.def("mlp_forward", &mlp_forward, "fused MLP forward (gfx950)",
        py::arg("x"), py::arg("weights"), py::arg("biases"), py::arg("acts"),
        py::arg("save_hidden"), py::arg("compute_bf16") = 0);
  m.def("mlp_backward", &mlp_backward, "fused MLP backward (gfx950)",
        py::arg("grad_out"), py::arg("x"), py::arg("weights"), py::arg("biases"),
        py::arg("hidden"), py::arg("final_out"), py::arg("acts"),
        py::arg("compute_bf16") = 0, py::arg("adam_m") = py::none(),
        py::arg("adam_v") = py::none(), py::arg("adam_step") = py::none(),
        py::arg("lr") = 0.0, py::arg("beta1") = 0.9, py::arg("beta2") = 0.999,
        py::arg("eps") = 1e-8, py::arg("weight_decay") = 0.0,
        py::arg("adam_step_delta") = 0.0, py::arg("adam_gate") = py::none(),
        py::arg("input_grad_only") = false);
  m.def("value_mlp_backward", &value_mlp_backward,
        "fused value-MSE whole-net backward (gfx950)", py::arg("x"),
        py::arg("weights"), py::arg("biases"), py::arg("hidden"),
        py::arg("final_out"), py::arg("acts"), py::arg("returns"),
        py::arg("compute_bf16") = 0, py::arg("partials_out") = py::none(),
        py::arg("adam_m") = py::none(), py::arg("adam_v") = py::none(),
        py::arg("adam_step") = py::none(), py::arg("lr") = 0.0,
        py::arg("beta1") = 0.9, py::arg("beta2") = 0.999,
        py::arg("eps") = 1e-8, py::arg("weight_decay") = 0.0,
        py::arg("adam_step_delta") = 0.0, py::arg("fwd_in_kernel") = false);
  m.def("value_loss_partials_blocks",
        [](int64_t batch) {
          return (batch + BWD_FUSED_ROWS - 1) / BWD_FUSED_ROWS;
        },
        "partials row length used by value_mlp_backward");
  m.def("value_loss_finalize", &value_loss_finalize,
        "batched deferred value-loss finalize (gfx950)");
  m.def("adam_bump_", &adam_bump_, "bump Adam step counters (gfx950)");
  m.def("adam_bump_dev_", &adam_bump_dev_,
        "bump Adam step counters by a device scalar (gfx950)");
  m.def("ppo_gate_update_", &ppo_gate_update_,
        "device-side KL early-stop gate bookkeeping (gfx950)");
  m.def("gaussian_ppo_policy_iter", &gaussian_ppo_policy_iter,
        "one 2-kernel Gaussian-PPO policy iteration (gfx950)");
  m.def("gaussian_ppo_value_twin_iter", &gaussian_ppo_value_twin_iter,
        "PPO policy + value iteration in one twin kernel pair (gfx950)");
  m.def("categorical_ppo_policy_iter", &categorical_ppo_policy_iter,
        "one 2-kernel categorical-PPO policy iteration (gfx950)");
  m.def("categorical_ppo_value_twin_iter", &categorical_ppo_value_twin_iter,
        "categorical-PPO policy + value iteration in one twin kernel pair "
        "(gfx950)");
  m.def("ppo_twin_uses_shaped", &ppo_twin_uses_shaped,
        "whether the twin iteration takes the [*,64,32,*] shaped kernel");
  m.def("reduce_adam_is_staged",
        [](int64_t n_blocks, int64_t grand) {
          return mlp_reduce_adam_is_staged((int)n_blocks, (long)grand);
        },
        "whether the reduce+Adam launch takes the LDS-staged kernel");
  m.def("segmented_gae", &segmented_gae, "segmented GAE+returns scan (gfx950)");
  m.def("normalize", &normalize, "fused mean/std normalize (gfx950)");
  m.def("q_target", &q_target, "fused Q-learning target (gfx950)");
  m.def("td3_smooth", &td3_smooth,
        "TD3 target-policy smoothing: Philox noise + clip + limit (gfx950)",
        py::arg("a"), py::arg("seed"), py::arg("offset"), py::arg("scale"),
        py::arg("clip"), py::arg("limit"), py::arg("offset_ctr") = py::none());
  m.def("q_target_min2", &q_target_min2,
        "fused min-twin Q-learning target (gfx950)");
  m.def("replay_gather", &replay_gather,
        "one-kernel Philox minibatch gather from the HBM replay ring (gfx950)",
        py::arg("obs"), py::arg("act"), py::arg("rew"), py::arg("nxt"),
        py::arg("dn"), py::arg("size_dev"), py::arg("B"), py::arg("seed"),
        py::arg("offset"), py::arg("offset_ctr") = py::none());
  m.def("fused_adam_", &fused_adam_, "fused multi-tensor Adam (gfx950)",
        py::arg("params"), py::arg("grads"), py::arg("exp_avgs"),
        py::arg("exp_avg_sqs"), py::arg("steps"), py::arg("lr"),
        py::arg("beta1"), py::arg("beta2"), py::arg("eps"),
        py::arg("weight_decay"), py::arg("step_delta") = 0.0,
        py::arg("do_bump") = true, py::arg("gate") = py::none());
  m.def("fused_polyak_", &fused_polyak_, "fused multi-tensor Polyak (gfx950)");
  m.def("gaussian_policy_loss", &gaussian_policy_loss,
        "fused Gaussian VPG/PPO loss fwd+bwd (gfx950)");
  m.def("gaussian_logp", &gaussian_logp, "Gaussian log-prob (gfx950)");
  m.def("gaussian_kl", &gaussian_kl, "approx KL for Gaussian policy (gfx950)");
  m.def("categorical_policy_loss", &categorical_policy_loss,
        "fused Categorical VPG/PPO loss fwd+bwd (gfx950)");
  m.def("categorical_logp", &categorical_logp, "Categorical log-prob (gfx950)");
  m.def("categorical_kl", &categorical_kl, "approx KL for Categorical policy (gfx950)");
  m.def("value_mse_loss", &value_mse_loss, "fused value MSE fwd+bwd (gfx950)");
  m.def("gaussian_sample", &gaussian_sample,
        "Philox Gaussian action sample (gfx950)", py::arg("mean"),
        py::arg("log_std"), py::arg("seed"), py::arg("offset"),
        py::arg("noise_scale"), py::arg("limit"),
        py::arg("offset_ctr") = py::none(), py::arg("out") = py::none());
  m.def("categorical_sample", &categorical_sample,
        "Philox categorical action sample (gfx950)", py::arg("logits"),
        py::arg("seed"), py::arg("offset"), py::arg("offset_ctr") = py::none(),
        py::arg("out") = py::none());
  m.def("synthetic_env_step", &synthetic_env_step,
        "fused synthetic-env transition + reward (gfx950)", py::arg("state"),
        py::arg("actions"), py::arg("A"), py::arg("B"), py::arg("w"),
        py::arg("sigma"), py::arg("seed"), py::arg("offset"),
        py::arg("do_reset"), py::arg("offset_ctr") = py::none(),
        py::arg("s_out") = py::none(), py::arg("final_out") = py::none(),
        py::arg("reward") = py::none());
  m.def("synthetic_env_reset", &synthetic_env_reset,
        "synthetic-env init states (gfx950)", py::arg("num_envs"),
        py::arg("obs_dim"), py::arg("like"), py::arg("seed"), py::arg("offset"),
        py::arg("offset_ctr") = py::none(), py::arg("out") = py::none());
  m.def("counter_add_", &counter_add_,
        "advance a device RNG counter (gfx950)");
}
```

rl_replicas_amd/ops/hip/common.h:

```cpp
#pragma once
#include <hip/hip_runtime.h>
#include <hip/hip_bf16.h>

#define WAVE 64
#define DEV_INLINE __device__ __forceinline__

typedef float f32x4 __attribute__((ext_vector_type(4)));
typedef __hip_bfloat16 bf16_t;
typedef __bf16 bf16x8 __attribute__((ext_vector_type(8)));

DEV_INLINE __bf16 f32_to_bf16(float v) {
  return (__bf16)v;
}

#define ACT_IDENTITY 0
#define ACT_TANH 1
#define ACT_RELU 2

DEV_INLINE float act_apply(int code, float x) {
  switch (code) {
    case ACT_TANH: return tanhf(x);
    case ACT_RELU: return x > 0.f ? x : 0.f;
    default: return x;
  }
}

DEV_INLINE float act_grad_from_y(int code, float y) {
  switch (code) {
    case ACT_TANH: return 1.f - y * y;
    case ACT_RELU: return y > 0.f ? 1.f : 0.f;
    default: return 1.f;
  }
}

#define LOG_2PI 1.8378770664093453f
DEV_INLINE float dlogp_coeff(int mode, float logp, float old_logp, float adv,
                             float clip, float* loss_out) {
  if (mode == 0) {
    *loss_out = -logp * adv;
    return -adv;
  }
  const float ratio = __expf(logp - old_logp);
  const float lo = 1.f - clip, hi = 1.f + clip;
  const float rc = fminf(fmaxf(ratio, lo), hi);
  const float s1 = ratio * adv;
  const float s2 = rc * adv;
  *loss_out = -fminf(s1, s2);
  const float g1 = (s1 < s2) ? 1.f : (s1 == s2 ? 0.5f : 0.f);
  const float inclip = (ratio >= lo && ratio <= hi) ? 1.f : 0.f;
  return -(g1 * s1 + (1.f - g1) * inclip * s1);
}

DEV_INLINE float row_lse(const float* logits, int n) {
  float m = logits[0];
  for (int j = 1; j < n; ++j) m = fmaxf(m, logits[j]);
  float s = 0.f;
  for (int j = 0; j < n; ++j) s += __expf(logits[j] - m);
  return m + __logf(s);
}

DEV_INLINE float wave_reduce_sum(float v) {
  #pragma unroll
  for (int off = 32; off > 0; off >>= 1) v += __shfl_down(v, off, 64);
  return v;
}

#define MLP_MAX_LAYERS 5
#define MLP_MAX_WIDTH 256
#define MLP_NARROW_WIDTH 64
#define MLP_LDS_BUDGET ((size_t)100 * 1024)
#define GAUSS_MAX_D 512

struct MLPArgs {
  const float* w[MLP_MAX_LAYERS];
  const float* b[MLP_MAX_LAYERS];
  float* h[MLP_MAX_LAYERS];
  int dims[MLP_MAX_LAYERS + 1];
  int acts[MLP_MAX_LAYERS];
  int n_layers;
  int batch;
};

struct MLPBwdArgs {
  const float* w[MLP_MAX_LAYERS];
  const float* h[MLP_MAX_LAYERS];
  const float* b[MLP_MAX_LAYERS];
  int dims[MLP_MAX_LAYERS + 1];
  int acts[MLP_MAX_LAYERS];
  int n_layers;
  int batch;
  long ws_stride;
  int layer_off[MLP_MAX_LAYERS];
};

struct ReduceAllArgs {
  const float* ws;
  long stride;
  float* dw[MLP_MAX_LAYERS];
  float* db[MLP_MAX_LAYERS];
  int total[MLP_MAX_LAYERS];
  int wsize[MLP_MAX_LAYERS];
  int n_layers;
  int n_blocks;
};

#define MT_MAX_TENSORS 16

struct AdamArgs {
  float* p[MT_MAX_TENSORS];
  float* g[MT_MAX_TENSORS];
  float* m[MT_MAX_TENSORS];
  float* v[MT_MAX_TENSORS];
  float* step[MT_MAX_TENSORS];
  int numel[MT_MAX_TENSORS];
  int n_tensors;
  float lr, beta1, beta2, eps, weight_decay;
  float step_delta;
  const float* gate;
};

struct PolyakArgs {
  const float* src[MT_MAX_TENSORS];
  float* dst[MT_MAX_TENSORS];
  int numel[MT_MAX_TENSORS];
  int n_tensors;
  float rho;
};

struct ReduceAdamArgs {
  const float* ws;
  long stride;
  float* pw[MLP_MAX_LAYERS];
  float* pb[MLP_MAX_LAYERS];
  float* mw[MLP_MAX_LAYERS];
  float* mb[MLP_MAX_LAYERS];
  float* vw[MLP_MAX_LAYERS];
  float* vb[MLP_MAX_LAYERS];
  const float* step;
  int total[MLP_MAX_LAYERS];
  int wsize[MLP_MAX_LAYERS];
  int n_layers, n_blocks;
  float lr, beta1, beta2, eps, weight_decay, step_delta;
  const float* gate;
  const float* kl_partials;
  const float* loss_partials;
  float* gate_rw;
  float* kl_final;
  float* iters_done;
  float* loss_out;
  float inv_b, thr;
  int first_iter;
};

#define SEED_GAUSSIAN 0
#define SEED_CATEGORICAL 1
struct GaussSeedArgs {
  const float* actions;
  const float* old_logp;
  const float* adv;
  const float* log_std;
  float* kl_partials;
  int dls_off;
  float clip;
  int kind;
  const float* skip_gate;
};

struct MLPBwdTwinArgs {
  MLPBwdArgs pol;
  GaussSeedArgs gauss;
  float* pol_ws;
  float* pol_loss_partials;
  MLPBwdArgs val;
  float* val_ws;
  const float* returns;
  float* val_loss_partials;
  const float* x;
};

#define ROLLOUT_ROWS 16
#define ROLLOUT_MAX_WIDTH 64
#define ROLLOUT_LDSW (ROLLOUT_MAX_WIDTH + 4)
#define ROLLOUT_MAX_CUTS 16
#define ROLLOUT_WIDE_LDSW (MLP_MAX_WIDTH + 4)

struct NetArgs {
  const float* w[MLP_MAX_LAYERS];
  const float* b[MLP_MAX_LAYERS];
  int dims[MLP_MAX_LAYERS + 1];
  int acts[MLP_MAX_LAYERS];
  int n_layers;
};

__host__ __device__ inline bool net_is_wide(const int* dims, int n_layers) {
  for (int l = 0; l <= n_layers; ++l)
    if (dims[l] > MLP_NARROW_WIDTH) return true;
  return false;
}

__host__ __device__ inline long net_lds_floats(int tiles, const int* dims,
                                               int n_layers) {
  if (net_is_wide(dims, n_layers)) return (long)tiles * ROLLOUT_ROWS * ROLLOUT_WIDE_LDSW;
  long n = (long)tiles * ROLLOUT_ROWS * ROLLOUT_LDSW;
  for (int l = 0; l < n_layers; ++l) n += dims[l + 1] * (dims[l] + 1) + dims[l + 1];
  return n;
}

struct RolloutFusedArgs : NetArgs {
  const float* log_std;
  const float* envA;
  const float* envB;
  const float* envw;
  float* obs_full;
  float* act_buf;
  float* rew_buf;
  float* cut_final;
  const unsigned long long* ctr;
  int cut_step[ROLLOUT_MAX_CUTS];
  int n_cuts;
  int N, O, A, steps;
  int start_with_reset;
  float sigma;
  uint64_t policy_seed, env_seed;
};

__host__ __device__ inline long rollout_fused_lds_floats(const int* dims, int n_layers,
                                                         int O, int A) {
  return net_lds_floats(5, dims, n_layers) + A + O * O + A * O + O;
}

struct CartPoleRolloutArgs : NetArgs {
  double* state;
  int* elapsed;
  float* obs_full;
  float* final_obs;
  long long* act_buf;
  float* rew_buf;
  unsigned char* done_buf;
  const unsigned long long* ctr;
  int N, steps, max_steps;
  int start_with_reset;
  uint64_t policy_seed, env_seed;
};

struct PendulumRolloutArgs : NetArgs {
  const float* log_std;
  double* state;
  float* obs_full;
  float* act_buf;
  float* rew_buf;
  float* cut_final;
  const unsigned long long* ctr;
  int cut_step[ROLLOUT_MAX_CUTS];
  int n_cuts;
  int N, steps;
  int start_with_reset;
  uint64_t policy_seed, env_seed;
};

struct ReplayRing {
  float* obs;
  float* act;
  float* rew;
  float* nxt;
  float* dn;
  const long long* write;
  unsigned long long cap;
};

#define COLLECT_NOISED 0
#define COLLECT_UNIFORM 1
struct PendulumCollectArgs : NetArgs {
  double* state;
  ReplayRing ring;
  float* seg_returns;
  float* last_obs;
  const unsigned long long* ctr;
  int cut_step[ROLLOUT_MAX_CUTS];
  int n_cuts, n_segs;
  int N, steps;
  int start_with_reset;
  int mode;
  float noise_scale, limit;
  float low, high;
  uint64_t action_seed, env_seed;
};

#define EVAL_DETERMINISTIC 0
#define EVAL_GAUSSIAN 1
struct PendulumEvalArgs : NetArgs {
  const float* log_std;
  double* returns;
  int* lengths;
  double* init_state;
  const unsigned long long* ctr;
  const unsigned long long* reset_ctr;
  int N, horizon;
  int mode;
  uint64_t policy_seed, env_seed;
};

struct CartPoleEvalArgs : NetArgs {
  double* returns;
  int* lengths;
  double* init_state;
  const unsigned long long* ctr;
  const unsigned long long* reset_ctr;
  int N, horizon;
  uint64_t policy_seed, env_seed;
};

struct ReplayScatterArgs {
  const float* obs_full;
  const float* act_buf;
  const float* rew_buf;
  const float* cut_final;
  const int* cut_slot;
  ReplayRing ring;
  float* seg_returns;
  int N, steps, n_cuts, n_segs;
};

struct ReplayGatherArgs {
  const float* obs;
  const float* act;
  const float* rew;
  const float* nxt;
  const float* dn;
  const long long* size;
  float* qin;
  float* obs_out;
  float* nxt_out;
  float* rew_out;
  float* dn_out;
  int B, O, A;
  uint64_t seed, offset;
  const unsigned long long* offset_ptr;
};
```

rl_replicas_amd/ops/hip/loss_kernels.hip:

```cpp
#include "common.h"

#define LOSS_THREADS 1024

DEV_INLINE float block_sum(float v, float* red ) {
  v = wave_reduce_sum(v);
  const int tid = threadIdx.x;
  if ((tid & 63) == 0) red[tid / WAVE] = v;
  __syncthreads();
  float total = 0.f;
  #pragma unroll
  for (int w = 0; w < LOSS_THREADS / WAVE; ++w) total += red[w];
  __syncthreads();
  return total;
}

#define LOSS_BLOCKS 32
#define LOSS_P_THREADS 256

template <int DT>
__global__ __launch_bounds__(LOSS_P_THREADS) void gaussian_policy_loss_bwd_t(
    const float* __restrict__ mean, const float* __restrict__ actions,
    const float* __restrict__ old_logp, const float* __restrict__ adv,
    const float* __restrict__ log_std, float* __restrict__ dmean,
    float* __restrict__ partials, int B, float clip, int mode) {
  __shared__ float red[LOSS_P_THREADS / WAVE];
  const int tid = threadIdx.x;
  const int gid = blockIdx.x * LOSS_P_THREADS + tid;

  float sigma[DT], inv_s2[DT];
  float base = 0.5f * (float)DT * LOG_2PI;
  #pragma unroll
  for (int d = 0; d < DT; ++d) {
    const float ls = log_std[d];
    sigma[d] = __expf(ls);
    inv_s2[d] = 1.f / (sigma[d] * sigma[d]);
    base += ls;
  }

  const float inv_b = 1.f / (float)B;
  float loss_acc = 0.f;
  float dls[DT];
  #pragma unroll
  for (int d = 0; d < DT; ++d) dls[d] = 0.f;

  for (int r = gid; r < B; r += gridDim.x * LOSS_P_THREADS) {
    float diff[DT];
    float q = 0.f;
    #pragma unroll
    for (int d = 0; d < DT; ++d) {
      diff[d] = actions[(long)r * DT + d] - mean[(long)r * DT + d];
      const float z = diff[d] / sigma[d];
      q += z * z;
    }
    const float logp = -0.5f * q - base;
    float loss_r;
    const float c = dlogp_coeff(mode, logp, old_logp ? old_logp[r] : 0.f,
                                adv[r], clip, &loss_r) * inv_b;
    loss_acc += loss_r * inv_b;
    #pragma unroll
    for (int d = 0; d < DT; ++d) {
      dmean[(long)r * DT + d] = c * diff[d] * inv_s2[d];
      const float z2 = diff[d] * diff[d] * inv_s2[d];
      dls[d] += c * (z2 - 1.f);
    }
  }

  #pragma unroll
  for (int d = 0; d < DT; ++d) {
    float v = wave_reduce_sum(dls[d]);
    if ((tid & 63) == 0) red[tid / WAVE] = v;
    __syncthreads();
    if (tid == 0) {
      float t = 0.f;
      for (int w = 0; w < LOSS_P_THREADS / WAVE; ++w) t += red[w];
      partials[(long)blockIdx.x * (DT + 1) + d] = t;
    }
    __syncthreads();
  }
  {
    float v = wave_reduce_sum(loss_acc);
    if ((tid & 63) == 0) red[tid / WAVE] = v;
    __syncthreads();
    if (tid == 0) {
      float t = 0.f;
      for (int w = 0; w < LOSS_P_THREADS / WAVE; ++w) t += red[w];
      partials[(long)blockIdx.x * (DT + 1) + DT] = t;
    }
  }
}

__global__ __launch_bounds__(LOSS_P_THREADS) void gaussian_policy_loss_bwd_g(
    const float* __restrict__ mean, const float* __restrict__ actions,
    const float* __restrict__ old_logp, const float* __restrict__ adv,
    const float* __restrict__ log_std, float* __restrict__ dmean,
    float* __restrict__ c_buf, float* __restrict__ partials, int B, int D,
    float clip, int mode) {
  __shared__ float red[LOSS_P_THREADS / WAVE];
  __shared__ float s_inv_s2[GAUSS_MAX_D];
  __shared__ float s_base;
  const int tid = threadIdx.x;
  for (int d = tid; d < D; d += LOSS_P_THREADS) {
    const float s = __expf(log_std[d]);
    s_inv_s2[d] = 1.f / (s * s);
  }
  if (tid == 0) {
    float b = 0.5f * (float)D * LOG_2PI;
    for (int d = 0; d < D; ++d) b += log_std[d];
    s_base = b;
  }
  __syncthreads();
  const float inv_b = 1.f / (float)B;
  float loss_acc = 0.f;
  for (int r = blockIdx.x * LOSS_P_THREADS + tid; r < B;
       r += gridDim.x * LOSS_P_THREADS) {
    float q = 0.f;
    for (int d = 0; d < D; ++d) {
      const float diff = actions[(long)r * D + d] - mean[(long)r * D + d];
      q += diff * diff * s_inv_s2[d];
    }
    const float logp = -0.5f * q - s_base;
    float loss_r;
    const float c = dlogp_coeff(mode, logp, old_logp ? old_logp[r] : 0.f,
                                adv[r], clip, &loss_r) * inv_b;
    c_buf[r] = c;
    loss_acc += loss_r * inv_b;
    for (int d = 0; d < D; ++d) {
      const float diff = actions[(long)r * D + d] - mean[(long)r * D + d];
      dmean[(long)r * D + d] = c * diff * s_inv_s2[d];
    }
  }
  __syncthreads();
  for (int d = 0; d < D; ++d) {
    float accd = 0.f;
    for (int r = blockIdx.x * LOSS_P_THREADS + tid; r < B;
         r += gridDim.x * LOSS_P_THREADS) {
      const float diff = actions[(long)r * D + d] - mean[(long)r * D + d];
      accd += c_buf[r] * (diff * diff * s_inv_s2[d] - 1.f);
    }
    float v = wave_reduce_sum(accd);
    if ((tid & 63) == 0) red[tid / WAVE] = v;
    __syncthreads();
    if (tid == 0) {
      float t = 0.f;
      for (int w = 0; w < LOSS_P_THREADS / WAVE; ++w) t += red[w];
      partials[(long)blockIdx.x * (D + 1) + d] = t;
    }
    __syncthreads();
  }
  {
    float v = wave_reduce_sum(loss_acc);
    if ((tid & 63) == 0) red[tid / WAVE] = v;
    __syncthreads();
    if (tid == 0) {
      float t = 0.f;
      for (int w = 0; w < LOSS_P_THREADS / WAVE; ++w) t += red[w];
      partials[(long)blockIdx.x * (D + 1) + D] = t;
    }
  }
}

__global__ void loss_partials_finalize(const float* __restrict__ partials,
                                       float* __restrict__ dlog_std,
                                       float* __restrict__ scalars, int n_blocks,
                                       int D) {
  const int d = threadIdx.x;
  if (d > D) return;
  float s = 0.f;
  for (int p = 0; p < n_blocks; ++p) s += partials[(long)p * (D + 1) + d];
  if (d < D) dlog_std[d] = s;
  else scalars[0] = s;
}

__global__ __launch_bounds__(256) void value_loss_finalize_rows(
    const float* __restrict__ partials, float* __restrict__ scalars, int rows,
    int fb, int row_stride) {
  const int lane = threadIdx.x & 63;
  const int r = blockIdx.x * 4 + (threadIdx.x >> 6);
  if (r >= rows) return;
  const float* row = partials + (long)r * row_stride;
  float s = 0.f;
  for (int p0 = 0; p0 < fb; p0 += 64) {
    const int v = p0 + lane < fb ? __float_as_int(row[p0 + lane]) : 0;
    const int n = min(64, fb - p0);
    for (int p = 0; p < n; ++p)
      s += __int_as_float(__builtin_amdgcn_readlane(v, p));
  }
  if (lane == 0) scalars[r] = s;
}

__global__ __launch_bounds__(LOSS_THREADS) void gaussian_logp_kernel(
    const float* __restrict__ mean, const float* __restrict__ actions,
    const float* __restrict__ log_std, float* __restrict__ logp, int B, int D) {
  const int tid = threadIdx.x + blockIdx.x * LOSS_THREADS;
  __shared__ float s_sigma[GAUSS_MAX_D];
  __shared__ float s_base;
  for (int d = threadIdx.x; d < D; d += LOSS_THREADS)
    s_sigma[d] = __expf(log_std[d]);
  if (threadIdx.x == 0) {
    float b = 0.f;
    for (int d = 0; d < D; ++d) b += log_std[d];
    s_base = b + 0.5f * (float)D * LOG_2PI;
  }
  __syncthreads();
  for (int r = tid; r < B; r += gridDim.x * LOSS_THREADS) {
    float q = 0.f;
    for (int d = 0; d < D; ++d) {
      const float z = (actions[(long)r * D + d] - mean[(long)r * D + d]) / s_sigma[d];
      q += z * z;
    }
    logp[r] = -0.5f * q - s_base;
  }
}

__global__ __launch_bounds__(LOSS_THREADS) void gaussian_kl_kernel(
    const float* __restrict__ mean, const float* __restrict__ actions,
    const float* __restrict__ log_std, const float* __restrict__ old_logp,
    float* __restrict__ out, int B, int D) {
  __shared__ float red[LOSS_THREADS / WAVE];
  __shared__ float s_sigma[GAUSS_MAX_D];
  const int tid = threadIdx.x;
  for (int d = tid; d < D; d += LOSS_THREADS) s_sigma[d] = __expf(log_std[d]);
  __syncthreads();
  float base = 0.f;
  for (int d = 0; d < D; ++d) base += log_std[d];
  base += 0.5f * (float)D * LOG_2PI;
  float acc = 0.f;
  for (int r = tid; r < B; r += LOSS_THREADS) {
    float q = 0.f;
    for (int d = 0; d < D; ++d) {
      const float z = (actions[(long)r * D + d] - mean[(long)r * D + d]) / s_sigma[d];
      q += z * z;
    }
    acc += old_logp[r] - (-0.5f * q - base);
  }
  const float total = block_sum(acc, red);
  if (tid == 0) out[0] = total / (float)B;
}

__global__ __launch_bounds__(LOSS_P_THREADS) void categorical_policy_loss_bwd(
    const float* __restrict__ logits, const float* __restrict__ actions,
    const float* __restrict__ old_logp, const float* __restrict__ adv,
    float* __restrict__ dlogits, float* __restrict__ partials, int B, int N,
    float clip, int mode) {
  __shared__ float red[LOSS_P_THREADS / WAVE];
  const int tid = threadIdx.x;
  const float inv_b = 1.f / (float)B;
  float loss_acc = 0.f;
  for (int r = blockIdx.x * LOSS_P_THREADS + tid; r < B;
       r += gridDim.x * LOSS_P_THREADS) {
    const float* lg = logits + (long)r * N;
    const int a = (int)actions[r];
    const float lse = row_lse(lg, N);
    const float logp = lg[a] - lse;
    float loss_r;
    const float c = dlogp_coeff(mode, logp, old_logp ? old_logp[r] : 0.f,
                                adv[r], clip, &loss_r) * inv_b;
    loss_acc += loss_r * inv_b;
    for (int j = 0; j < N; ++j) {
      const float p = __expf(lg[j] - lse);
      dlogits[(long)r * N + j] = c * (((j == a) ? 1.f : 0.f) - p);
    }
  }
  float v = wave_reduce_sum(loss_acc);
  if ((tid & 63) == 0) red[tid / WAVE] = v;
  __syncthreads();
  if (tid == 0) {
    float t = 0.f;
    for (int w = 0; w < LOSS_P_THREADS / WAVE; ++w) t += red[w];
    partials[blockIdx.x] = t;
  }
}

__global__ __launch_bounds__(LOSS_THREADS) void categorical_logp_kernel(
    const float* __restrict__ logits, const float* __restrict__ actions,
    float* __restrict__ logp, int B, int N) {
  const int tid = threadIdx.x + blockIdx.x * LOSS_THREADS;
  for (int r = tid; r < B; r += gridDim.x * LOSS_THREADS) {
    const float* lg = logits + (long)r * N;
    logp[r] = lg[(int)actions[r]] - row_lse(lg, N);
  }
}

__global__ __launch_bounds__(LOSS_THREADS) void categorical_kl_kernel(
    const float* __restrict__ logits, const float* __restrict__ actions,
    const float* __restrict__ old_logp, float* __restrict__ out, int B, int N) {
  __shared__ float red[LOSS_THREADS / WAVE];
  const int tid = threadIdx.x;
  float acc = 0.f;
  for (int r = tid; r < B; r += LOSS_THREADS) {
    const float* lg = logits + (long)r * N;
    acc += old_logp[r] - (lg[(int)actions[r]] - row_lse(lg, N));
  }
  const float total = block_sum(acc, red);
  if (tid == 0) out[0] = total / (float)B;
}

void launch_gaussian_loss(const float* mean, const float* actions,
                          const float* old_logp, const float* adv,
                          const float* log_std, float* dmean, float* c_buf,
                          float* partials, int B, int D, float clip, int mode,
                          int n_blocks, hipStream_t stream) {
  dim3 g(n_blocks), b(LOSS_P_THREADS);
#define CASE_D(DT)                                                           \
  case DT:                                                                   \
    hipLaunchKernelGGL((gaussian_policy_loss_bwd_t<DT>), g, b, 0, stream,    \
                       mean, actions, old_logp, adv, log_std, dmean,         \
                       partials, B, clip, mode);                             \
    break;
  switch (D) {
    CASE_D(1) CASE_D(2) CASE_D(3) CASE_D(4)
    CASE_D(5) CASE_D(6) CASE_D(7) CASE_D(8)
    default:
      hipLaunchKernelGGL(gaussian_policy_loss_bwd_g, g, b, 0, stream, mean,
                         actions, old_logp, adv, log_std, dmean, c_buf,
                         partials, B, D, clip, mode);
      break;
  }
#undef CASE_D
}

__global__ __launch_bounds__(LOSS_THREADS) void value_mse_bwd_kernel(
    const float* __restrict__ v, const float* __restrict__ ret,
    float* __restrict__ dv, float* __restrict__ scalars, int B) {
  __shared__ float red[LOSS_THREADS / WAVE];
  const int tid = threadIdx.x;
  const float inv_b = 1.f / (float)B;
  float loss_acc = 0.f;
  for (int r = tid; r < B; r += LOSS_THREADS) {
    const float diff = v[r] - ret[r];
    loss_acc += diff * diff * inv_b;
    dv[r] = 2.f * diff * inv_b;
  }
  const float loss = block_sum(loss_acc, red);
  if (tid == 0) scalars[0] = loss;
}
```

rl_replicas_amd/ops/hip/rollout_steps.h:

```cpp
#pragma once
#include <hip/hip_runtime.h>

#include "common.h"
#include "philox.h"

template <int LDSW, bool BF16>
DEV_INLINE f32x4 mlp_fwd_tile_lds(const float* buf_in, const float* wl, int wrow,
                                  int in_d, int arow, int k, int j, bool jok) {
  f32x4 acc = {0.f, 0.f, 0.f, 0.f};
  if constexpr (BF16) {
    for (int k0 = 0; k0 < in_d; k0 += 32) {
      bf16x8 af, bf;
      #pragma unroll
      for (int e = 0; e < 8; ++e) {
        const int kk = k0 + k * 8 + e;
        af[e] = f32_to_bf16((kk < in_d) ? buf_in[arow * LDSW + kk] : 0.f);
        bf[e] = f32_to_bf16((jok && kk < in_d) ? wl[j * wrow + kk] : 0.f);
      }
      acc = __builtin_amdgcn_mfma_f32_16x16x32_bf16(af, bf, acc, 0, 0, 0);
    }
  } else {
    for (int k0 = 0; k0 < in_d; k0 += 4) {
      const int kk = k0 + k;
      float a = (kk < in_d) ? buf_in[arow * LDSW + kk] : 0.f;
      float bv = (jok && kk < in_d) ? wl[j * wrow + kk] : 0.f;
      acc = __builtin_amdgcn_mfma_f32_16x16x4f32(a, bv, acc, 0, 0, 0);
    }
  }
  return acc;
}

template <int LDSW>
DEV_INLINE void mlp_fwd_tile_epilogue(f32x4 acc, const float* B, int act, int j,
                                      bool jok, int wr0, int lane, float* buf_out) {
  if (jok) {
    const float bias = B[j];
    #pragma unroll
    for (int r = 0; r < 4; ++r) {
      const int row = wr0 + (lane >> 4) * 4 + r;
      buf_out[row * LDSW + j] = act_apply(act, acc[r] + bias);
    }
  }
}

template <int LDSW>
DEV_INLINE f32x4 mlp_fwd_tile_wide(const float* xt, const float* wrow, int in_d,
                                   int i, int k, bool jok) {
  const int in4 = in_d & ~3;
  const int in8 = in_d & ~7;
  f32x4 acc = {0.f, 0.f, 0.f, 0.f};
  f32x4 acc2 = {0.f, 0.f, 0.f, 0.f};
  for (int k0 = 0; k0 < in8; k0 += 8) {
    float bv0 = 0.f, bv1 = 0.f;
    if (jok) {
      bv0 = wrow[k0 + k];
      bv1 = wrow[k0 + 4 + k];
    }
    const float a0 = xt[i * LDSW + k0 + k];
    const float a1 = xt[i * LDSW + k0 + 4 + k];
    acc = __builtin_amdgcn_mfma_f32_16x16x4f32(a0, bv0, acc, 0, 0, 0);
    acc2 = __builtin_amdgcn_mfma_f32_16x16x4f32(a1, bv1, acc2, 0, 0, 0);
  }
  for (int k0 = in8; k0 < in4; k0 += 4) {
    float bv = jok ? wrow[k0 + k] : 0.f;
    const float a = xt[i * LDSW + k0 + k];
    acc = __builtin_amdgcn_mfma_f32_16x16x4f32(a, bv, acc, 0, 0, 0);
  }
  if (in4 < in_d) {
    const int kk = in4 + k;
    float a = (kk < in_d) ? xt[i * LDSW + kk] : 0.f;
    float bv = (jok && kk < in_d) ? wrow[kk] : 0.f;
    acc = __builtin_amdgcn_mfma_f32_16x16x4f32(a, bv, acc, 0, 0, 0);
  }
  acc[0] += acc2[0]; acc[1] += acc2[1]; acc[2] += acc2[2]; acc[3] += acc2[3];
  return acc;
}


struct NetStage {
  const float* bl;
  float* end;
};

template <int NT, bool WIDE>
DEV_INLINE NetStage net_stage(const NetArgs& a, float* wl, int tid) {
  if constexpr (WIDE) return {nullptr, wl};
  int woff = 0;
  for (int l = 0; l < a.n_layers; ++l) {
    const int in_d = a.dims[l], out_d = a.dims[l + 1];
    for (int idx = tid; idx < out_d * in_d; idx += NT) {
      const int r = idx / in_d, c = idx % in_d;
      wl[woff + r * (in_d + 1) + c] = a.w[l][idx];
    }
    woff += out_d * (in_d + 1);
  }
  float* const bl = wl + woff;
  int boff = 0;
  for (int l = 0; l < a.n_layers; ++l) {
    for (int idx = tid; idx < a.dims[l + 1]; idx += NT) bl[boff + idx] = a.b[l][idx];
    boff += a.dims[l + 1];
  }
  return {bl, bl + boff};
}

template <int NT, int LDSW, bool WIDE>
DEV_INLINE const float* net_forward(const NetArgs& a, const float* st, float* buf0,
                                    float* buf1, const float* wl, const float* bl,
                                    int wave, int lane) {
  constexpr int NW = NT / 64;
  const int i16 = lane & 15;
  const int k4 = lane >> 4;
  const float* buf_in = st;
  int wo = 0, bo = 0;
  for (int l = 0; l < a.n_layers; ++l) {
    const int in_d = a.dims[l], out_d = a.dims[l + 1];
    float* const buf_out = (l & 1) ? buf1 : buf0;
    for (int jt = wave * 16; jt < out_d; jt += 16 * NW) {
      const int j = jt + i16;
      const bool jok = j < out_d;
      if constexpr (WIDE) {
        const f32x4 acc = mlp_fwd_tile_wide<LDSW>(buf_in, a.w[l] + (long)j * in_d,
                                                  in_d, i16, k4, jok);
        mlp_fwd_tile_epilogue<LDSW>(acc, a.b[l], a.acts[l], j, jok, 0, lane, buf_out);
      } else {
        const f32x4 acc = mlp_fwd_tile_lds<LDSW, false>(buf_in, wl + wo, in_d + 1,
                                                        in_d, i16, k4, j, jok);
        mlp_fwd_tile_epilogue<LDSW>(acc, bl + bo, a.acts[l], j, jok, 0, lane, buf_out);
      }
    }
    __syncthreads();
    buf_in = buf_out;
    wo += out_d * (in_d + 1);
    bo += out_d;
  }
  return buf_in;
}

DEV_INLINE int cut_slot(const int* cut_step, int n_cuts, int t) {
  int slot = -1;
  for (int c = 0; c < n_cuts; ++c)
    if (cut_step[c] == t) slot = c;
  return slot;
}

DEV_INLINE float uniform_sample_elem(float low, float high, uint64_t seed,
                                     uint64_t offset, uint32_t i) {
  uint32_t r[4];
  philox4(seed, offset, i, r);
  return low + (high - low) * u32_to_open_unit(r[0]);
}

DEV_INLINE unsigned long long ring_slot(unsigned long long write,
                                        unsigned long long cap, int row, int steps,
                                        int t) {
  return (write + (unsigned long long)row * (unsigned long long)steps +
          (unsigned long long)t) % cap;
}

DEV_INLINE float gaussian_sample_elem(float mean, const float* log_std, int d,
                                      uint64_t seed, uint64_t offset, uint32_t i,
                                      float noise_scale, float limit) {
  uint32_t r[4];
  philox4(seed, offset, i, r);
  float z0, z1;
  box_muller(r[0], r[1], &z0, &z1);
  const float sigma = noise_scale >= 0.f ? noise_scale : __expf(log_std[d]);
  float a = mean + sigma * z0;
  if (limit >= 0.f) a = fminf(fmaxf(a, -limit), limit);
  return a;
}

DEV_INLINE void synthetic_env_row(const float* s, const float* a, const float* A,
                                  const float* Bm, const float* w, int row, int o,
                                  int O, int Adim, float sigma, uint64_t seed,
                                  uint64_t offset, int do_reset, float* out_o_p,
                                  float* s_next_p, float* rsum_p) {
  float r_part = 0.f;
  float out_o = 0.f;
  if (o < O) {
    float acc = 0.f;
    for (int k = 0; k < O; ++k) acc += s[k] * A[k * O + o];
    for (int j = 0; j < Adim; ++j) {
      const float aj = fminf(fmaxf(a[j], -1.f), 1.f);
      acc += aj * Bm[j * O + o];
    }
    if (sigma > 0.f)
      acc += sigma * philox_normal(seed, offset, (uint32_t)(row * O + o));
    out_o = tanhf(acc);
    r_part = out_o * w[o];
  }
  if (o == 0) {
    float pen = 0.f;
    for (int j = 0; j < Adim; ++j) {
      const float aj = fminf(fmaxf(a[j], -1.f), 1.f);
      pen += aj * aj;
    }
    r_part -= 0.1f * pen;
  }
  *rsum_p = wave_reduce_sum(r_part);
  float s_next = out_o;
  if (o < O && do_reset) {
    s_next = 0.1f * philox_normal(seed, offset + 1, (uint32_t)(row * O + o));
  }
  *out_o_p = out_o;
  *s_next_p = s_next;
}

DEV_INLINE int categorical_sample_row(const float* lg, int n, uint64_t seed,
                                      uint64_t offset, uint32_t row) {
  float m = lg[0];
  for (int j = 1; j < n; ++j) m = fmaxf(m, lg[j]);
  float z = 0.f;
  for (int j = 0; j < n; ++j) z += __expf(lg[j] - m);
  uint32_t r[4];
  philox4(seed, offset, row, r);
  const float u = u32_to_open_unit(r[0]) * z;
  float acc = 0.f;
  int pick = n - 1;
  for (int j = 0; j < n; ++j) {
    acc += __expf(lg[j] - m);
    if (u <= acc) { pick = j; break; }
  }
  return pick;
}

DEV_INLINE bool cartpole_row_step(double s[4], int action) {
#pragma clang fp contract(off)
  constexpr double GRAVITY = 9.8;
  constexpr double MASSPOLE = 0.1;
  constexpr double TOTAL_MASS = 1.0 + 0.1;
  constexpr double LENGTH = 0.5;
  constexpr double POLEMASS_LENGTH = 0.1 * 0.5;
  constexpr double FORCE_MAG = 10.0;
  constexpr double TAU = 0.02;
  constexpr double THETA_THRESHOLD = 24.0 * 3.141592653589793 / 360.0;
  constexpr double X_THRESHOLD = 2.4;
  double x = s[0], x_dot = s[1], theta = s[2], theta_dot = s[3];
  const double force = action == 1 ? FORCE_MAG : -FORCE_MAG;
  const double costheta = cos(theta);
  const double sintheta = sin(theta);
  const double temp =
      (force + POLEMASS_LENGTH * (theta_dot * theta_dot) * sintheta) / TOTAL_MASS;
  const double thetaacc =
      (GRAVITY * sintheta - costheta * temp) /
      (LENGTH * (4.0 / 3.0 - MASSPOLE * (costheta * costheta) / TOTAL_MASS));
  const double xacc = temp - POLEMASS_LENGTH * thetaacc * costheta / TOTAL_MASS;
  x = x + TAU * x_dot;
  x_dot = x_dot + TAU * xacc;
  theta = theta + TAU * theta_dot;
  theta_dot = theta_dot + TAU * thetaacc;
  s[0] = x; s[1] = x_dot; s[2] = theta; s[3] = theta_dot;
  return fabs(x) > X_THRESHOLD || fabs(theta) > THETA_THRESHOLD;
}

DEV_INLINE void cartpole_reset_draw(uint64_t seed, uint64_t offset, uint32_t row,
                                    double out[4]) {
#pragma clang fp contract(off)
  uint32_t r[4];
  philox4(seed, offset, row, r);
  #pragma unroll
  for (int k = 0; k < 4; ++k)
    out[k] = -0.05 + 0.1 * (((double)r[k] + 0.5) * (1.0 / 4294967296.0));
}

DEV_INLINE bool cartpole_env_row(double s[4], int* elapsed, int action,
                                 int max_steps, uint64_t seed, uint64_t offset,
                                 uint32_t row, float fin[4], float obs[4]) {
  const bool terminated = cartpole_row_step(s, action);
  const int el = *elapsed + 1;
  const bool truncated = max_steps > 0 && el >= max_steps && !terminated;
  const bool done = terminated || truncated;
  #pragma unroll
  for (int k = 0; k < 4; ++k) fin[k] = (float)s[k];
  if (done) cartpole_reset_draw(seed, offset, row, s);
  *elapsed = done ? 0 : el;
  #pragma unroll
  for (int k = 0; k < 4; ++k) obs[k] = (float)s[k];
  return done;
}

DEV_INLINE void pendulum_row_step(double s[2], float action, float* reward) {
#pragma clang fp contract(off)
  constexpr double PI = 3.141592653589793;
  constexpr double TWO_PI = 2.0 * 3.141592653589793;
  constexpr double MAX_SPEED = 8.0;
  constexpr double MAX_TORQUE = 2.0;
  constexpr double DT = 0.05;
  const double th = s[0], thdot = s[1];
  const double u = fmin(fmax((double)action, -MAX_TORQUE), MAX_TORQUE);
  double ang = fmod(th + PI, TWO_PI);
  if (ang < 0.0) ang = ang + TWO_PI;
  ang = ang - PI;
  const double costs = ang * ang + 0.1 * (thdot * thdot) + 0.001 * (u * u);
  double newthdot = thdot + (15.0 * sin(th) + 3.0 * u) * DT;
  newthdot = fmin(fmax(newthdot, -MAX_SPEED), MAX_SPEED);
// ... 35 lines not shown
```

rl_replicas_amd/ops/hip/update_kernels.hip:

```cpp
#include "common.h"

#define MT_CHUNK 8192

__global__ __launch_bounds__(256) void fused_adam_kernel(AdamArgs a) {
  if (a.gate && *a.gate == 0.f) return;
  const int t = blockIdx.x;
  if (t >= a.n_tensors) return;
  const int n = a.numel[t];
  const int c0 = blockIdx.y * MT_CHUNK;
  if (c0 >= n) return;
  const int c1 = min(c0 + MT_CHUNK, n);
  const float s = a.step[t][0] + 1.f + a.step_delta;
  const float bc1 = 1.f - __powf(a.beta1, s);
  const float bc2 = 1.f - __powf(a.beta2, s);

  float* p = a.p[t];
  float* g = a.g[t];
  float* m = a.m[t];
  float* v = a.v[t];
  for (int i = c0 + threadIdx.x; i < c1; i += 256) {
    float grad = g[i];
    if (a.weight_decay != 0.f) grad += a.weight_decay * p[i];
    float mi = a.beta1 * m[i] + (1.f - a.beta1) * grad;
    float vi = a.beta2 * v[i] + (1.f - a.beta2) * grad * grad;
    m[i] = mi;
    v[i] = vi;
    const float mhat = mi / bc1;
    const float vhat = vi / bc2;
    p[i] -= a.lr * mhat / (sqrtf(vhat) + a.eps);
  }
}

__global__ void adam_step_bump_kernel(AdamArgs a) {
  if (a.gate && *a.gate == 0.f) return;
  const int t = threadIdx.x;
  if (t < a.n_tensors) a.step[t][0] += a.step_delta;
}

__global__ void adam_step_bump_dev_kernel(AdamArgs a,
                                          const float* __restrict__ amount) {
  const int t = threadIdx.x;
  if (t < a.n_tensors) a.step[t][0] += *amount;
}

__global__ void ppo_gate_update_kernel(float* gate, const float* kl,
                                       float* kl_final, float* iters_done,
                                       float thr) {
  if (*gate != 0.f) {
    *kl_final = *kl;
    *iters_done += 1.f;
    if (*kl > thr) *gate = 0.f;
  }
}

__global__ __launch_bounds__(256) void fused_polyak_kernel(PolyakArgs a) {
  const int t = blockIdx.x;
  if (t >= a.n_tensors) return;
  const int n = a.numel[t];
  const int c0 = blockIdx.y * MT_CHUNK;
  if (c0 >= n) return;
  const int c1 = min(c0 + MT_CHUNK, n);
  const float* s = a.src[t];
  float* d = a.dst[t];
  const float rho = a.rho, one_m = 1.f - a.rho;
  for (int i = c0 + threadIdx.x; i < c1; i += 256) {
    d[i] = rho * d[i] + one_m * s[i];
  }
}
```

rl_replicas_amd/samplers/device_sampler.py:

```python
from __future__ import annotations

from typing import Dict, List, Optional, Tuple

import numpy as np
import torch

from rl_replicas_amd.envs.device import DevicePendulumEnv, DeviceVectorEnv
from rl_replicas_amd.experience import Experience
from rl_replicas_amd.policies import Policy
from rl_replicas_amd.samplers.sampler import Sampler


def lockstep_cuts(steps: int, horizon: Optional[int], start_elapsed: int) -> Tuple[int, ...]:
    if horizon is None:
        return ()
    return tuple(t for t in range(steps) if (start_elapsed + t + 1) % horizon == 0)


def segment_bounds(steps: int, cuts: Tuple[int, ...]) -> List[tuple]:
    bounds: List[tuple] = []
    start = 0
    for c in cuts:
        bounds.append((start, c + 1, True))
        start = c + 1
    if start < steps:
        bounds.append((start, steps, False))
    return bounds


def cached_graph(sampler, key: tuple, build):
    g = sampler._graphs.get(key)
    if g is None:
        if sampler._graph_ctr is None:
            from rl_replicas_amd.ops import fused_rollout

            sampler._graph_ctr = fused_rollout.make_counter(sampler.env.device)
        g = sampler._graphs[key] = build(sampler._graph_ctr)
    return g


class DeviceSampler(Sampler):
    def __init__(self, device_env: DeviceVectorEnv, seed: Optional[int] = None, is_continuous: bool = False):
        self.env = device_env
        self.seed = seed
        self.is_continuous = is_continuous
        self.num_envs = device_env.num_envs
        self._obs: Optional[torch.Tensor] = None
        self._bufs = None
        self._graphs: Dict[tuple, object] = {}
        self._graph_ctr: Optional[torch.Tensor] = None

    def _get_bufs(self, steps: int, obs_dim: int, act_dim: int, device):
        if self._bufs is None or self._bufs[0].shape[0] != steps:
            N = self.num_envs
            self._bufs = (
                torch.empty(steps, N, obs_dim, device=device),
                torch.empty(steps, N, act_dim, device=device),
                torch.empty(steps, N, device=device),
            )
        return self._bufs

    def sample(self, num_samples: int, policy: Policy) -> Experience:
        env = self.env
        N = self.num_envs
        if num_samples % N != 0:
            raise ValueError(
                f"num_samples ({num_samples}) must be divisible by num_envs ({N})"
            )
        steps = num_samples // N
        obs_dim = int(env.observation_space.shape[0])
        act_dim = int(env.action_space.shape[0])

        first = self._obs is None
        reset_epoch = first or not self.is_continuous
        horizon = env.spec.max_episode_steps
        start_elapsed = 0 if reset_epoch else env._elapsed
        cuts = lockstep_cuts(steps, horizon, start_elapsed)

        from rl_replicas_amd.ops import fused_rollout

        pendulum = isinstance(env, DevicePendulumEnv)
        can_graph = (fused_rollout.pendulum_supported(policy, env) if pendulum
                     else fused_rollout.supported(policy, env))
        graph_ok = can_graph and (
            (steps, cuts, reset_epoch) in self._graphs or len(self._graphs) < 8
        )
        if graph_ok:
            if first and self.seed is not None:
                env.seed(self.seed)
            obs_buf, act_buf, rew_buf, finals = self._sample_graphed(
                policy, steps, cuts, reset_epoch
            )
        else:
            obs_buf, act_buf, rew_buf, finals = self._sample_eager(
                policy, steps, cuts, reset_epoch, obs_dim, act_dim
            )
        env._elapsed = steps - (cuts[-1] + 1) if cuts else start_elapsed + steps

        return self._build_experience(
            steps, cuts, obs_buf, act_buf, rew_buf, finals, obs_dim, act_dim
        )

    def _sample_graphed(self, policy, steps: int, cuts: Tuple[int, ...],
                        reset_epoch: bool):
        from rl_replicas_amd.ops import fused_rollout

        env = self.env
        pendulum = isinstance(env, DevicePendulumEnv)
        cls = (fused_rollout.GraphedPendulumRollout if pendulum
               else fused_rollout.GraphedRollout)
        g = cached_graph(
            self, (steps, cuts, reset_epoch),
            lambda ctr: cls(policy, env, steps, cuts, reset_epoch, ctr),
        )
        if not pendulum and not reset_epoch:
            g.obs_full[steps].copy_(self._obs)
        g.replay()
        self._obs = g.obs_full[steps]
        if not pendulum:
            env.state = self._obs
        return g.obs_full[:steps], g.act_buf, g.rew_buf, g.final_tensors()

    def _sample_eager(self, policy, steps: int, cuts: Tuple[int, ...],
                      reset_epoch: bool, obs_dim: int, act_dim: int):
        env = self.env
        if self._obs is None:
            self._obs = env.reset(seed=self.seed)
        elif reset_epoch:
            self._obs = env.reset()
        obs_buf, act_buf, rew_buf = self._get_bufs(steps, obs_dim, act_dim, env.device)

        finals: List[torch.Tensor] = []
        obs = self._obs
        for t in range(steps):
            obs_buf[t].copy_(obs)
            actions = policy.get_action_tensor(obs).to(
                device=obs.device, dtype=torch.float32
            )
            act_buf[t].copy_(actions)
            obs, reward, truncated, final_obs = env.step(actions)
            rew_buf[t].copy_(reward)
            if truncated:
                finals.append(final_obs)
        assert len(finals) == len(cuts)
        self._obs = obs
        return obs_buf, act_buf, rew_buf, finals

    def _build_experience(self, steps: int, cuts: Tuple[int, ...], obs_buf,
                          act_buf, rew_buf, finals, obs_dim: int,
                          act_dim: int) -> Experience:
        N = self.num_envs
        device = self.env.device

        seg_bounds = segment_bounds(steps, cuts)
        n_segs = len(seg_bounds)

        flat_obs = torch.empty(N * steps, obs_dim, device=device)
        flat_act = torch.empty(N * steps, act_dim, device=device)
        flat_rew = torch.empty(N * steps, device=device)
        flat_obs.view(N, steps, obs_dim).copy_(obs_buf.transpose(0, 1))
        flat_act.view(N, steps, act_dim).copy_(act_buf.transpose(0, 1))
        rew_t = flat_rew.view(N, steps)
        rew_t.copy_(rew_buf.transpose(0, 1))

        lasts = [finals[j] if done else self._obs for j, (_, _, done) in enumerate(seg_bounds)]
        last_obs = torch.stack(lasts, dim=1).reshape(N * n_segs, obs_dim)

        seg_lengths = [e - s for s, e, _ in seg_bounds]
        offsets_np = np.zeros(N * n_segs + 1, dtype=np.int32)
        np.cumsum(np.tile(seg_lengths, N), out=offsets_np[1:])
        dones_pattern = [d for _, _, d in seg_bounds]

        seg_returns = torch.stack(
            [rew_t[:, s:e].sum(dim=1) for s, e, _ in seg_bounds], dim=1
        ).cpu().numpy()

        flat_next = torch.empty(N * steps, obs_dim, device=device)
        nv = flat_next.view(N, steps, obs_dim)
        if steps > 1:
            nv[:, : steps - 1].copy_(obs_buf[1:].transpose(0, 1))
        nv[:, steps - 1].copy_(self._obs)
        step_dones = torch.zeros(N, steps, device=device)
        for j, c in enumerate(cuts):
            nv[:, c].copy_(finals[j])
            step_dones[:, c] = 1.0

        experience = Experience()
        experience.episode_returns = [float(r) for r in seg_returns.reshape(-1)]
        experience.episode_lengths = seg_lengths * N
        experience.dones = [
            np.concatenate([np.zeros(L - 1, dtype=bool), [d]])
            for L, d in zip(seg_lengths, dones_pattern)
        ] * N
        experience.set_flat_cache(
            {
                "observations": flat_obs,
                "actions": flat_act,
                "rewards": flat_rew,
                "episode_offsets": torch.as_tensor(offsets_np, device=device),
                "episode_dones": torch.as_tensor(
                    np.tile(dones_pattern, N), device=device
                ),
                "last_observations": last_obs,
                "next_observations": flat_next,
                "step_dones": step_dones.reshape(-1),
            }
        )
        return experience
```

setup.py:

```python
import os

from setuptools import setup

os.environ.setdefault("PYTORCH_ROCM_ARCH", "gfx950")

from torch.utils.cpp_extension import BuildExtension, CUDAExtension

HIP_DIR = os.path.join("rl_replicas_amd", "ops", "hip")

ext = CUDAExtension(
    name="rl_replicas_amd._hip_ops",
    sources=[
        os.path.join(HIP_DIR, "bindings.hip"),
        os.path.join(HIP_DIR, "mlp_kernels.hip"),
        os.path.join(HIP_DIR, "loss_kernels.hip"),
        os.path.join(HIP_DIR, "sample_kernels.hip"),
        os.path.join(HIP_DIR, "env_kernels.hip"),
        os.path.join(HIP_DIR, "rollout_kernels.hip"),
        os.path.join(HIP_DIR, "rollout_fused_kernels.hip"),
        os.path.join(HIP_DIR, "cartpole_rollout_kernels.hip"),
        os.path.join(HIP_DIR, "pendulum_rollout_kernels.hip"),
        os.path.join(HIP_DIR, "pendulum_collect_kernels.hip"),
        os.path.join(HIP_DIR, "eval_kernels.hip"),
        os.path.join(HIP_DIR, "update_kernels.hip"),
        os.path.join(HIP_DIR, "offpolicy_kernels.hip"),
    ],
    extra_compile_args={
        "cxx": ["-O3", "-std=c++17"],
        "nvcc": ["-O3", "-std=c++17", "--offload-arch=gfx950"],
    },
)

setup(
    name="rl_replicas_amd",
    version="0.1.0",
    packages=[
        "rl_replicas",
        "rl_replicas_amd",
        "rl_replicas_amd.algorithms",
        "rl_replicas_amd.envs",
        "rl_replicas_amd.networks",
        "rl_replicas_amd.ops",
        "rl_replicas_amd.optimizers",
        "rl_replicas_amd.parallel",
        "rl_replicas_amd.policies",
        "rl_replicas_amd.samplers",
    ],
    ext_modules=[ext],
    cmdclass={"build_ext": BuildExtension},
)
```

Measured before the change: 1.576 million env-steps/s.

## Graph-capture whole PPO epoch with fused ingest kernel and on-device epilogue

```diff
diff --git a/rl_replicas_amd/algorithms/on_policy.py b/rl_replicas_amd/algorithms/on_policy.py
--- a/rl_replicas_amd/algorithms/on_policy.py
+++ b/rl_replicas_amd/algorithms/on_policy.py
@@ -69,6 +69,9 @@
         self.metrics_manager.close()
 
     def _prepare_batch(self, experience: Experience) -> Dict[str, Tensor]:
+        return self._finish_batch(*self._upload_batch(experience), self.device)
+
+    def _upload_batch(self, experience: Experience):
         device = self.device
         flat = experience.to_flat_batch()
         if isinstance(flat["observations"], Tensor):
@@ -76,7 +79,7 @@
             actions = flat["actions"].to(device=device, dtype=torch.float32)
             rewards = flat["rewards"].to(device)
             last_obs = flat["last_observations"].to(device)
-            return self._finish_batch(flat, obs, actions, rewards, last_obs, device)
+            return flat, obs, actions, rewards, last_obs
         obs_np = flat["observations"]
         act_np = np.asarray(flat["actions"], dtype=np.float32)
         rew_np = flat["rewards"]
@@ -107,7 +110,7 @@
             actions = torch.as_tensor(act_np, device=device)
             rewards = torch.as_tensor(rew_np, dtype=torch.float32, device=device)
             last_obs = torch.as_tensor(last_np, dtype=torch.float32, device=device)
-        return self._finish_batch(flat, obs, actions, rewards, last_obs, device)
+        return flat, obs, actions, rewards, last_obs
 
     def _finish_batch(self, flat, obs, actions, rewards, last_obs, device) -> Dict[str, Tensor]:
         offsets = torch.as_tensor(flat["episode_offsets"], device=device)
@@ -140,13 +143,16 @@
         return ops.normalize(advantages)
 
     def train(self, experience: Experience) -> None:
-        batch = self._prepare_batch(experience)
-        obs = batch["observations"]
-        actions = batch["actions"]
-        advantages = batch["advantages"]
-        returns = batch["discounted_returns"]
-
-        joint = self._update_policy_and_value(obs, actions, advantages, returns)
+        uploaded = self._upload_batch(experience)
+        joint = self._train_epoch_fused(*uploaded)
+        if joint is None:
+            batch = self._finish_batch(*uploaded, self.device)
+            obs = batch["observations"]
+            actions = batch["actions"]
+            advantages = batch["advantages"]
+            returns = batch["discounted_returns"]
+
+            joint = self._update_policy_and_value(obs, actions, advantages, returns)
         if joint is not None:
             policy_metrics, value_loss = joint
         else:
@@ -166,6 +172,10 @@
     def _update_policy(self, obs: Tensor, actions: Tensor, advantages: Tensor) -> Dict[str, float]:
         raise NotImplementedError
 
+    def _train_epoch_fused(self, flat, obs: Tensor, actions: Tensor, rewards: Tensor,
+                           last_obs: Tensor):
+        return None
+
     def _update_policy_and_value(self, obs: Tensor, actions: Tensor, advantages: Tensor,
                                  returns: Tensor):
         return None
diff --git a/rl_replicas_amd/algorithms/ppo.py b/rl_replicas_amd/algorithms/ppo.py
--- a/rl_replicas_amd/algorithms/ppo.py
+++ b/rl_replicas_amd/algorithms/ppo.py
@@ -68,6 +68,15 @@
             "policy/kl_divergence": float(approximate_kl),
         }
 
+    def _train_epoch_fused(self, flat, obs: Tensor, actions: Tensor, rewards: Tensor,
+                           last_obs: Tensor):
+        from rl_replicas_amd import ops
+        from rl_replicas_amd.ops import fused_onpolicy
+
+        if not (obs.is_cuda and ops.hip_available()):
+            return None
+        return fused_onpolicy.ppo_epoch_update(self, flat, obs, actions, rewards, last_obs)
+
     def _update_policy_and_value(self, obs: Tensor, actions: Tensor, advantages: Tensor,
                                  returns: Tensor):
         from rl_replicas_amd.ops import fused_onpolicy
diff --git a/rl_replicas_amd/ops/fused_onpolicy.py b/rl_replicas_amd/ops/fused_onpolicy.py
--- a/rl_replicas_amd/ops/fused_onpolicy.py
+++ b/rl_replicas_amd/ops/fused_onpolicy.py
@@ -532,26 +532,45 @@
 
     def __init__(self, algo, obs0: Tensor, actions0: Tensor, adv0: Tensor,
                  old_logp0: Tensor, returns0: Tensor):
-        from rl_replicas_amd.ops.fused_adam import adam_arg_lists
-
-        ext = ops._load_extension()
-        policy, vf = algo.policy, algo.value_function
-        pmlp, vmlp = _mlp_of(policy), vf.network
         dev = obs0.device
         self.obs = obs0.clone()
         self.actions = actions0.clone()
         self.adv = adv0.clone()
         self.old_logp = old_logp0.clone()
         self.returns = returns0.clone()
-        clip = float(algo.clip_range)
-        thr = 1.5 * float(algo.max_kl_divergence)
-        num_p = int(algo.num_policy_gradients)
-        num_v = int(algo.num_value_gradients)
-        assert 1 <= num_p <= num_v
         self.gate = torch.ones(1, device=dev)
         self.kl_final = torch.zeros(1, device=dev)
         self.loss0 = torch.zeros(1, device=dev)
         self.iters_done = torch.zeros(1, device=dev)
+        self._capture(algo)
+
+    def _head(self) -> None:
+        self.gate.fill_(1.0)
+        self.iters_done.zero_()
+
+    def _tail(self, algo, kl: Tensor) -> Tensor:
+        ext = ops._load_extension()
+        ext.ppo_gate_update_(self.gate, kl, self.kl_final, self.iters_done,
+                             self._thr)
+        algo.policy.optimizer.bump_steps_by(self.iters_done)
+        algo.value_function.optimizer.bump_steps(float(self._num_v))
+        return ext.value_loss_finalize(self.partials, self._fb)
+
+    def _extra_state(self, algo) -> List[Tensor]:
+        return []
+
+    def _capture(self, algo) -> None:
+        from rl_replicas_amd.ops.fused_adam import adam_arg_lists
+
+        ext = ops._load_extension()
+        policy, vf = algo.policy, algo.value_function
+        pmlp, vmlp = _mlp_of(policy), vf.network
+        dev = self.obs.device
+        clip = float(algo.clip_range)
+        thr = self._thr = 1.5 * float(algo.max_kl_divergence)
+        num_p = int(algo.num_policy_gradients)
+        num_v = self._num_v = int(algo.num_value_gradients)
+        assert 1 <= num_p <= num_v
         scratch_loss = torch.zeros(1, device=dev)
 
         pw, pb, pacts = _extract_layers(pmlp)
@@ -568,13 +587,12 @@
         vm, vv, vstep, vhp = adam_arg_lists(vf.optimizer, vw, vb)
         state += [p.data for p in vf.parameters()]
         state += _ensure_adam_state(vf.optimizer)
-        fb = int(ext.value_loss_partials_blocks(obs0.shape[0]))
+        fb = self._fb = int(ext.value_loss_partials_blocks(self.obs.shape[0]))
         self.partials = torch.zeros(num_v, fb, device=dev)
         dummy = torch.empty(0, device=dev)
 
         def body():
-            self.gate.fill_(1.0)
-            self.iters_done.zero_()
+            self._head()
             for i in range(num_p):
                 twin_iter(
                     self.obs, list(pw), list(pb), pacts, self.actions,
@@ -597,13 +615,9 @@
                                      self.old_logp)
             else:
                 kl = ext.categorical_kl(out, self.actions, self.old_logp)
-            ext.ppo_gate_update_(self.gate, kl, self.kl_final,
-                                 self.iters_done, thr)
-            policy.optimizer.bump_steps_by(self.iters_done)
-            vf.optimizer.bump_steps(float(num_v))
-            return ext.value_loss_finalize(self.partials, fb)
-
-        self.loop = _CapturedLoop(body, state)
+            return self._tail(algo, kl)
+
+        self.loop = _CapturedLoop(body, state + self._extra_state(algo))
 
     def run(self, algo, obs, actions, advantages, old_logp, returns):
         self.obs.copy_(obs)
@@ -622,6 +636,180 @@
             "policy/loss": float(self.loss0[0]),
             "policy/kl_divergence": float(self.kl_final[0]),
         }, float(losses.mean())
+
+
+class _GraphedPPOEpoch(_GraphedPPOTwin):
+
+    GATE, KL, LOSS0, ITERS_LIVE, ITERS, LOG_STD_SUM, LOGP_STD, VALUE_LOSS = range(8)
+
+    def __init__(self, algo, obs: Tensor, actions: Tensor, rewards: Tensor,
+                 last_obs: Tensor, offsets: Tensor, dones: Tensor):
+        dev = obs.device
+        T, E = obs.shape[0], last_obs.shape[0]
+        self.obs = torch.empty_like(obs)
+        self.actions = torch.empty_like(actions)
+        self.rewards = torch.empty(T, device=dev)
+        self.offsets = torch.empty(E + 1, dtype=torch.int32, device=dev)
+        self.dones = torch.empty(E, dtype=torch.int32, device=dev)
+        self.values_all = torch.empty(T + E, device=dev)
+        self.old_logp = torch.empty(T, device=dev)
+        self.logp_now = torch.empty(T, device=dev)
+        self.adv_raw = torch.empty(T, device=dev)
+        self.adv = torch.empty(T, device=dev)
+        self.returns = torch.empty(T, device=dev)
+        self.losses = torch.empty(int(algo.num_value_gradients), device=dev)
+        self.metrics = torch.zeros(8, device=dev)
+        self.metrics[self.GATE] = 1.0
+        self.gate = self.metrics[self.GATE:self.GATE + 1]
+        self.kl_final = self.metrics[self.KL:self.KL + 1]
+        self.loss0 = self.metrics[self.LOSS0:self.LOSS0 + 1]
+        self.iters_done = self.metrics[self.ITERS_LIVE:self.ITERS_LIVE + 1]
+        self.ingest(algo, obs, actions, rewards, last_obs, offsets, dones)
+        self._capture(algo)
+
+    def ingest(self, algo, obs, actions, rewards, last_obs, offsets, dones) -> None:
+        ext = ops._load_extension()
+        policy, old = algo.policy, algo.old_policy
+        vw, vb, vacts = _extract_layers(algo.value_function.network)
+        pw, pb, pacts = _extract_layers(_mlp_of(policy))
+        ow, ob, _ = _extract_layers(_mlp_of(old))
+        ext.ppo_ingest_rows(
+            obs, last_obs, actions, rewards, offsets, dones,
+            list(vw), list(vb), vacts, list(pw), list(pb), pacts,
+            policy.log_std.data, list(ow), list(ob), old.log_std.data,
+            self.obs, self.actions, self.rewards, self.offsets, self.dones,
+            self.values_all, self.old_logp, self.logp_now,
+        )
+
+    def _head(self) -> None:
+        ext = ops._load_extension()
+        ext.segmented_gae_out(self.rewards, self.values_all, self.offsets,
+                              self.dones, self._gamma, self._lam, self.adv_raw,
+                              self.returns)
+        ext.normalize_out(self.adv_raw, self.adv)
+        torch.sum(self._log_std, dim=0, out=self.metrics[self.LOG_STD_SUM])
+        torch.std(self.logp_now, dim=0, out=self.metrics[self.LOGP_STD])
+
+    def _tail(self, algo, kl: Tensor) -> Tensor:
+        ext = ops._load_extension()
+        policy, vf = algo.policy, algo.value_function
+        src = policy.state_dict()
+        dst = algo.old_policy.state_dict()
+        assert list(src) == list(dst)
+        ext.ppo_epoch_epilogue_(
+            self.gate, kl, self.kl_final, self.iters_done,
+            self.metrics[self.ITERS:self.ITERS + 1], self._thr,
+            _step_counters(policy.optimizer), _step_counters(vf.optimizer),
+            float(self._num_v), self.partials, self._fb, self.losses,
+            list(src.values()), list(dst.values()),
+        )
+        torch.mean(self.losses, dim=0, out=self.metrics[self.VALUE_LOSS])
+        return self.losses
+
+    def _extra_state(self, algo) -> List[Tensor]:
+        return [self.metrics] + [p.data for p in algo.old_policy.parameters()]
+
+    def _capture(self, algo) -> None:
+        self._gamma, self._lam = float(algo.gamma), float(algo.gae_lambda)
+        self._log_std = algo.policy.log_std.detach()
+        super()._capture(algo)
+
+    def run(self, algo, obs, actions, rewards, last_obs, offsets, dones):
+        self.ingest(algo, obs, actions, rewards, last_obs, offsets, dones)
+        self.loop.replay()
+        m = self.metrics.cpu()
+        iters = int(m[self.ITERS])
+        if iters < algo.num_policy_gradients:
+            logger.info(
+                "Early stopping at update %d due to reaching max KL divergence.",
+                iters - 1,
+            )
+        d = algo.policy.log_std.numel()
+        entropy = float(m[self.LOG_STD_SUM]) + 0.5 * d * (1.0 + math.log(2 * math.pi))
+        return {
+            "policy/loss": float(m[self.LOSS0]),
+            "policy/avarage_entropy": entropy,
+            "policy/log_prob_std": float(m[self.LOGP_STD]),
+            "policy/kl_divergence": float(m[self.KL]),
+        }, float(m[self.VALUE_LOSS])
+
+
+def _step_counters(optimizer) -> List[Tensor]:
+    return [
+        optimizer.state[p]["step"]
+        for group in optimizer.param_groups
+        for p in group["params"]
+        if p in optimizer.state and "step" in optimizer.state[p]
+    ]
+
+
+EPOCH_GRAPH_CACHE = 8
+
+
+def _epoch_graph_enabled() -> bool:
+    return os.environ.get("RL_REPLICAS_AMD_PPO_EPOCH_GRAPH", "1") != "0"
+
+
+def ppo_epoch_eligible(algo, obs: Tensor) -> bool:
+    from rl_replicas_amd.algorithms.on_policy import OnPolicyAlgorithm
+
+    if not _epoch_graph_enabled() or ops.compute_bf16() != 0:
+        return False
+    if getattr(algo, "_dp_replicate", False) or getattr(algo, "_dp_enabled", False):
+        return False
+    for hook in ("_gather_global_batch", "_normalize_advantages"):
+        if getattr(type(algo), hook) is not getattr(OnPolicyAlgorithm, hook) \
+                or hook in vars(algo):
+            return False
+    if not (obs.is_cuda and obs.dtype == torch.float32 and obs.dim() == 2):
+        return False
+    if _policy_kind(algo.policy) != "gaussian" or not ppo_twin_eligible(algo, obs):
+        return False
+    old_mlp = _mlp_of(getattr(algo, "old_policy", None) or algo.policy)
+    if old_mlp is None or _extract_layers(old_mlp) is None:
+        return False
+    ext = ops._load_extension()
+    max_width, budget = ext.ppo_ingest_rows_limits()
+    dims = []
+    for mlp in (algo.value_function.network, _mlp_of(algo.policy), old_mlp):
+        weights = _extract_layers(mlp)[0]
+        dims.append([int(weights[0].shape[1])] + [int(w.shape[0]) for w in weights])
+    vdims, pdims, odims = dims
+    if odims != pdims or max(vdims + pdims) > max_width:
+        return False
+    return int(ext.ppo_ingest_rows_lds_bytes(vdims, pdims)) <= budget
+
+
+def ppo_epoch_update(algo, flat, obs: Tensor, actions: Tensor, rewards: Tensor,
+                     last_obs: Tensor):
+    if not ppo_epoch_eligible(algo, obs):
+        return None
+    policy = algo.policy
+    obs = obs.contiguous()
+    actions = actions.contiguous().view(obs.shape[0], -1)
+    if actions.shape[1] != policy.log_std.numel() or last_obs.shape[0] < 1:
+        return None
+    rewards = rewards.contiguous()
+    last_obs = last_obs.contiguous()
+    dev = obs.device
+    offsets = torch.as_tensor(flat["episode_offsets"], device=dev).to(torch.int32)
+    dones = torch.as_tensor(flat["episode_dones"], device=dev).to(torch.int32)
+    key = (tuple(obs.shape), tuple(actions.shape), int(last_obs.shape[0]),
+           int(algo.num_policy_gradients), int(algo.num_value_gradients),
+           float(algo.gamma), float(algo.gae_lambda),
+           tuple(id(p) for p in policy.parameters()),
+           tuple(id(p) for p in algo.value_function.parameters()),
+           tuple(id(p) for p in algo.old_policy.parameters()))
+    graphs = algo.__dict__.setdefault("_ppo_epoch_graphs", {})
+    graphed = graphs.get(key)
+    if graphed is None:
+        if len(graphs) >= EPOCH_GRAPH_CACHE:
+            return None
+        graphed = graphs[key] = _GraphedPPOEpoch(
+            algo, obs, actions, rewards, last_obs, offsets, dones
+        )
+    algo.epoch_graph_replays = getattr(algo, "epoch_graph_replays", 0) + 1
+    return graphed.run(algo, obs, actions, rewards, last_obs, offsets, dones)
 
 
 def _get_cached_graph(algo, attr: str, key, builder):
diff --git a/rl_replicas_amd/ops/hip/bindings.hip b/rl_replicas_amd/ops/hip/bindings.hip
--- a/rl_replicas_amd/ops/hip/bindings.hip
+++ b/rl_replicas_amd/ops/hip/bindings.hip
@@ -127,6 +127,8 @@
 __global__ void counter_add_kernel(unsigned long long* ctr,
                                    unsigned long long delta);
 void launch_ppo_rollout_fused(const RolloutFusedArgs& a, hipStream_t stream);
+void launch_ppo_ingest_rows(const PPOIngestArgs& a, hipStream_t stream);
+__global__ void ppo_epoch_epilogue(PPOEpilogueArgs a);
 __global__ void segmented_gae_kernel(const float* rewards, const float* values,
                                      const float* last_values, const int* offsets,
                                      const int* dones, float* advantages,
@@ -788,6 +790,17 @@
   return out;
 }
 
+static void launch_segmented_gae(const float* rewards, const float* values,
+                                 const float* last_values, const int* offsets,
+                                 const int* dones, float* adv, float* ret, int n_eps,
+                                 double gamma, double lam) {
+  if (n_eps <= 0) return;
+  hipLaunchKernelGGL(segmented_gae_kernel, dim3(n_eps), dim3(256), 0,
+                     current_stream(), rewards, values, last_values, offsets, dones,
+                     adv, ret, (float)gamma, (float)lam);
+  HIP_OK(hipGetLastError());
+}
+
 std::vector<torch::Tensor> segmented_gae(torch::Tensor rewards, torch::Tensor values,
                                          torch::Tensor last_values,
                                          torch::Tensor offsets, torch::Tensor dones,
@@ -800,25 +813,55 @@
   const int n_eps = (int)last_values.size(0);
   auto adv = torch::empty_like(rewards);
   auto ret = torch::empty_like(rewards);
-  if (n_eps > 0) {
-    hipLaunchKernelGGL(segmented_gae_kernel, dim3(n_eps), dim3(256), 0,
-                       current_stream(), rewards.data_ptr<float>(),
-                       values.data_ptr<float>(), last_values.data_ptr<float>(),
-                       offsets.data_ptr<int>(), dones.data_ptr<int>(),
-                       adv.data_ptr<float>(), ret.data_ptr<float>(), (float)gamma,
-                       (float)lam);
-    HIP_OK(hipGetLastError());
-  }
+  launch_segmented_gae(rewards.data_ptr<float>(), values.data_ptr<float>(),
+                       last_values.data_ptr<float>(), offsets.data_ptr<int>(),
+                       dones.data_ptr<int>(), adv.data_ptr<float>(),
+                       ret.data_ptr<float>(), n_eps, gamma, lam);
   return {adv, ret};
+}
+
+void segmented_gae_out(torch::Tensor rewards, torch::Tensor values_all,
+                       torch::Tensor offsets, torch::Tensor dones, double gamma,
+                       double lam, torch::Tensor adv, torch::Tensor ret) {
+  check_f32_gpu(rewards, "rewards");
+  check_f32_gpu(values_all, "values_all");
+  check_f32_gpu(adv, "adv");
+  check_f32_gpu(ret, "ret");
+  const int64_t T = rewards.numel();
+  const int64_t n_eps = values_all.numel() - T;
+  TORCH_CHECK(n_eps >= 0 && adv.numel() == T && ret.numel() == T,
+              "segmented_gae_out: rewards/adv/ret [T], values_all [T + E]");
+  TORCH_CHECK(offsets.scalar_type() == torch::kInt32 && offsets.is_cuda() &&
+                  offsets.is_contiguous() && offsets.numel() == n_eps + 1,
+              "offsets must be a contiguous int32 GPU tensor [E + 1]");
+  TORCH_CHECK(dones.scalar_type() == torch::kInt32 && dones.is_cuda() &&
+                  dones.is_contiguous() && dones.numel() == n_eps,
+              "dones must be a contiguous int32 GPU tensor [E]");
+  launch_segmented_gae(rewards.data_ptr<float>(), values_all.data_ptr<float>(),
+                       values_all.data_ptr<float>() + T, offsets.data_ptr<int>(),
+                       dones.data_ptr<int>(), adv.data_ptr<float>(),
+                       ret.data_ptr<float>(), (int)n_eps, gamma, lam);
+}
+
+static void launch_normalize(const torch::Tensor& x, torch::Tensor& y) {
+  hipLaunchKernelGGL(normalize_kernel, dim3(1), dim3(1024), 0, current_stream(),
+                     x.data_ptr<float>(), y.data_ptr<float>(), (int)x.numel());
+  HIP_OK(hipGetLastError());
 }
 
 torch::Tensor normalize(torch::Tensor x) {
   check_f32_gpu(x, "x");
   auto y = torch::empty_like(x);
-  hipLaunchKernelGGL(normalize_kernel, dim3(1), dim3(1024), 0, current_stream(),
-                     x.data_ptr<float>(), y.data_ptr<float>(), (int)x.numel());
-  HIP_OK(hipGetLastError());
+  launch_normalize(x, y);
   return y;
+}
+
+void normalize_out(torch::Tensor x, torch::Tensor y) {
+  check_f32_gpu(x, "x");
+  check_f32_gpu(y, "y");
+  TORCH_CHECK(y.numel() == x.numel() && y.data_ptr() != x.data_ptr(),
+              "normalize_out: y must be a second buffer of x's size");
+  launch_normalize(x, y);
 }
 
 torch::Tensor q_target(torch::Tensor r, torch::Tensor d, torch::Tensor qn,
@@ -923,6 +966,70 @@
                      rows, (int)fb, stride);
   HIP_OK(hipGetLastError());
   return scalars;
+}
+
+void ppo_epoch_epilogue_(torch::Tensor gate, torch::Tensor kl, torch::Tensor kl_final,
+                         torch::Tensor iters_done, torch::Tensor iters_out,
+                         double thr, std::vector<torch::Tensor> pol_steps,
+                         std::vector<torch::Tensor> val_steps, double val_bump,
+                         torch::Tensor partials, int64_t fb, torch::Tensor losses,
+                         std::vector<torch::Tensor> srcs,
+                         std::vector<torch::Tensor> dsts) {
+  PPOEpilogueArgs a{};
+  for (const torch::Tensor* t : {&gate, &kl, &kl_final, &iters_done, &iters_out}) {
+    check_f32_gpu(*t, "gate/kl/kl_final/iters_done/iters_out");
+    TORCH_CHECK(t->numel() >= 1, "gate bookkeeping scalars must not be empty");
+  }
+  TORCH_CHECK(gate.numel() == 1 && kl_final.numel() == 1 && iters_done.numel() == 1 &&
+                  iters_out.numel() == 1,
+              "gate bookkeeping scalars must have 1 element");
+  a.gate = gate.data_ptr<float>();
+  a.kl = kl.data_ptr<float>();
+  a.kl_final = kl_final.data_ptr<float>();
+  a.iters_done = iters_done.data_ptr<float>();
+  a.iters_out = iters_out.data_ptr<float>();
+  a.thr = (float)thr;
+  TORCH_CHECK(pol_steps.size() <= MT_MAX_TENSORS && val_steps.size() <= MT_MAX_TENSORS &&
+                  srcs.size() <= MT_MAX_TENSORS && srcs.size() == dsts.size(),
+              "ppo_epoch_epilogue_: at most ", MT_MAX_TENSORS,
+              " step counters per optimizer and synced tensors");
+  auto fill_steps = [](const std::vector<torch::Tensor>& steps, float** out) {
+    for (size_t i = 0; i < steps.size(); ++i) {
+      TORCH_CHECK(steps[i].is_cuda() && steps[i].scalar_type() == torch::kFloat32 &&
+                      steps[i].numel() == 1,
+                  "adam step must be a 1-element fp32 GPU tensor");
+      out[i] = steps[i].data_ptr<float>();
+    }
+  };
+  fill_steps(pol_steps, a.pol_step);
+  fill_steps(val_steps, a.val_step);
+  a.n_pol_steps = (int)pol_steps.size();
+  a.n_val_steps = (int)val_steps.size();
+  a.val_bump = (float)val_bump;
+  check_f32_gpu(partials, "partials");
+  check_f32_gpu(losses, "losses");
+  TORCH_CHECK(partials.dim() == 2, "partials must be [rows, stride]");
+  a.rows = (int)partials.size(0);
+  a.row_stride = (int)partials.size(1);
+  a.fb = (int)fb;
+  TORCH_CHECK(fb >= 0 && a.fb <= a.row_stride, "fb exceeds partials row stride");
+  TORCH_CHECK(losses.numel() == a.rows, "losses must hold one element per row");
+  a.partials = partials.data_ptr<float>();
+  a.losses = losses.data_ptr<float>();
+  a.n_sync = (int)srcs.size();
+  for (int i = 0; i < a.n_sync; ++i) {
+    check_f32_gpu(srcs[i], "sync source");
+    check_f32_gpu(dsts[i], "sync destination");
+    TORCH_CHECK(srcs[i].numel() == dsts[i].numel() &&
+                    srcs[i].numel() < (1LL << 31),
+                "sync source and destination differ in size");
+    a.src[i] = srcs[i].data_ptr<float>();
+    a.dst[i] = dsts[i].data_ptr<float>();
+    a.numel[i] = (int)srcs[i].numel();
+  }
+  hipLaunchKernelGGL(ppo_epoch_epilogue, dim3((a.rows + 3) / 4 + 1 + a.n_sync),
+                     dim3(256), 0, current_stream(), a);
+  HIP_OK(hipGetLastError());
 }
 
 void fused_polyak_(std::vector<torch::Tensor> srcs, std::vector<torch::Tensor> dsts,
@@ -1902,6 +2009,102 @@
   a.action_seed = (uint64_t)action_seed;
   a.env_seed = (uint64_t)env_seed;
   launch_pendulum_collect_fused(a, (int)wide_threads, current_stream());
+  HIP_OK(hipGetLastError());
+}
+
+static size_t ppo_ingest_lds_bytes(const NetLayout& v, const NetLayout& p) {
+  return (size_t)ppo_ingest_lds_floats(v.dims, v.L, p.dims, p.L) * sizeof(float);
+}
+
+int64_t ppo_ingest_rows_lds_bytes_py(std::vector<int64_t> vdims,
+                                     std::vector<int64_t> pdims) {
+  return (int64_t)ppo_ingest_lds_bytes(net_layout(vdims, ROLLOUT_MAX_WIDTH),
+                                       net_layout(pdims, ROLLOUT_MAX_WIDTH));
+}
+
+void ppo_ingest_rows(torch::Tensor observations, torch::Tensor last_observations,
+                     torch::Tensor actions, torch::Tensor rewards,
+                     torch::Tensor offsets, torch::Tensor dones,
+                     std::vector<torch::Tensor> vweights,
+                     std::vector<torch::Tensor> vbiases, std::vector<int64_t> vacts,
+                     std::vector<torch::Tensor> pweights,
+                     std::vector<torch::Tensor> pbiases, std::vector<int64_t> pacts,
+                     torch::Tensor log_std, std::vector<torch::Tensor> oweights,
+                     std::vector<torch::Tensor> obiases, torch::Tensor old_log_std,
+                     torch::Tensor obs_out, torch::Tensor act_out,
+                     torch::Tensor rew_out, torch::Tensor off_out,
+                     torch::Tensor dones_out, torch::Tensor values_all,
+                     torch::Tensor old_logp, torch::Tensor logp_now) {
+  PPOIngestArgs a{};
+  const NetLayout pnet =
+      net_layout(observations, pweights, pbiases, pacts, ROLLOUT_MAX_WIDTH);
+  const NetLayout onet =
+      net_layout(observations, oweights, obiases, pacts, ROLLOUT_MAX_WIDTH);
+  const NetLayout vnet =
+      net_layout(observations, vweights, vbiases, vacts, ROLLOUT_MAX_WIDTH);
+  TORCH_CHECK(onet.L == pnet.L, "the old policy must have the policy's shape");
+  for (int l = 0; l <= pnet.L; ++l)
+    TORCH_CHECK(onet.dims[l] == pnet.dims[l], "the old policy must have the policy's shape");
+  TORCH_CHECK(vnet.dims[vnet.L] == 1, "ppo_ingest_rows: the value head must be 1 wide");
+  const torch::Device dev = observations.device();
+  check_net_device(pweights, pbiases, dev);
+  check_net_device(oweights, obiases, dev);
+  check_net_device(vweights, vbiases, dev);
+  TORCH_CHECK(ppo_ingest_lds_bytes(vnet, pnet) <= MLP_LDS_BUDGET,
+              "ppo_ingest_rows: net images exceed the LDS budget");
+
+  const int64_t T = observations.size(0), O = observations.size(1);
+  const int64_t A = pnet.dims[pnet.L];
+  check_f32_gpu(last_observations, "last_observations");
+  TORCH_CHECK(last_observations.dim() == 2 && last_observations.size(1) == O,
+              "last_observations must be [E, O]");
+  const int64_t E = last_observations.size(0);
+  TORCH_CHECK(T >= 1 && E >= 1 && T + E < (1LL << 24), "row count out of range");
+  for (const torch::Tensor* t : {&actions, &rewards, &log_std, &old_log_std})
+    check_f32_gpu(*t, "actions / rewards / log_std");
+  TORCH_CHECK(actions.numel() == T * A && rewards.numel() == T,
+              "actions must be [T, A] and rewards [T]");
+  TORCH_CHECK(log_std.numel() == A && old_log_std.numel() == A, "log_std must be [A]");
+  check_out(offsets, torch::kInt32, E + 1, "offsets");
+  check_out(dones, torch::kInt32, E, "dones");
+  check_out(obs_out, torch::kFloat32, T * O, "obs_out");
+  check_out(act_out, torch::kFloat32, T * A, "act_out");
+  check_out(rew_out, torch::kFloat32, T, "rew_out");
+  check_out(off_out, torch::kInt32, E + 1, "off_out");
+  check_out(dones_out, torch::kInt32, E, "dones_out");
+  check_out(values_all, torch::kFloat32, T + E, "values_all");
+  check_out(old_logp, torch::kFloat32, T, "old_logp");
+  check_out(logp_now, torch::kFloat32, T, "logp_now");
+  for (const torch::Tensor* t :
+       {&last_observations, &actions, &rewards, &offsets, &dones, &log_std,
+        &old_log_std, &obs_out, &act_out, &rew_out, &off_out, &dones_out,
+        &values_all, &old_logp, &logp_now})
+    TORCH_CHECK(t->device() == dev, "ppo_ingest_rows: tensors on different devices");
+
+  fill_net(a.val, vnet, vweights, vbiases, vacts);
+  fill_net(a.pol, pnet, pweights, pbiases, pacts);
+  fill_net(a.old, onet, oweights, obiases, pacts);
+  a.obs = observations.data_ptr<float>();
+  a.last_obs = last_observations.data_ptr<float>();
+  a.actions = actions.data_ptr<float>();
+  a.rewards = rewards.data_ptr<float>();
+  a.offsets = offsets.data_ptr<int>();
+  a.dones = dones.data_ptr<int>();
+  a.log_std = log_std.data_ptr<float>();
+  a.old_log_std = old_log_std.data_ptr<float>();
+  a.obs_out = obs_out.data_ptr<float>();
+  a.act_out = act_out.data_ptr<float>();
+  a.rew_out = rew_out.data_ptr<float>();
+  a.off_out = off_out.data_ptr<int>();
+  a.dones_out = dones_out.data_ptr<int>();
+  a.values_all = values_all.data_ptr<float>();
+  a.old_logp = old_logp.data_ptr<float>();
+  a.logp_now = logp_now.data_ptr<float>();
+  a.T = (int)T;
+  a.E = (int)E;
+  a.O = (int)O;
+  a.A = (int)A;
+  launch_ppo_ingest_rows(a, current_stream());
   HIP_OK(hipGetLastError());
 }
 
@@ -2313,6 +2516,22 @@
         "whether the reduce+Adam launch takes the LDS-staged kernel");
   m.def("segmented_gae", &segmented_gae, "segmented GAE+returns scan (gfx950)");
   m.def("normalize", &normalize, "fused mean/std normalize (gfx950)");
+  m.def("segmented_gae_out", &segmented_gae_out,
+        "segmented GAE+returns scan into the caller's buffers (gfx950)");
+  m.def("normalize_out", &normalize_out,
+        "fused mean/std normalize into the caller's buffer (gfx950)");
+  m.def("ppo_ingest_rows", &ppo_ingest_rows,
+        "one pass over a PPO epoch's rows: three forwards, two log-probs and "
+        "the copies into the update graph's buffers (gfx950)");
+  m.def("ppo_ingest_rows_lds_bytes", &ppo_ingest_rows_lds_bytes_py,
+        "dynamic LDS of ppo_ingest_rows for (value dims, policy dims)");
+  m.def("ppo_ingest_rows_limits",
+        []() {
+          return std::vector<int64_t>{ROLLOUT_MAX_WIDTH, (int64_t)MLP_LDS_BUDGET};
+        },
+        "(max width, LDS budget) of ppo_ingest_rows");
+  m.def("ppo_epoch_epilogue_", &ppo_epoch_epilogue_,
+        "the captured PPO epoch's tail in one launch (gfx950)");
   m.def("q_target", &q_target, "fused Q-learning target (gfx950)");
   m.def("td3_smooth", &td3_smooth,
         "TD3 target-policy smoothing: Philox noise + clip + limit (gfx950)",
diff --git a/rl_replicas_amd/ops/hip/common.h b/rl_replicas_amd/ops/hip/common.h
--- a/rl_replicas_amd/ops/hip/common.h
+++ b/rl_replicas_amd/ops/hip/common.h
@@ -63,6 +63,20 @@
   #pragma unroll
   for (int off = 32; off > 0; off >>= 1) v += __shfl_down(v, off, 64);
   return v;
+}
+
+DEV_INLINE void value_loss_row_sum(const float* __restrict__ partials,
+                                   float* __restrict__ scalars, int r, int fb,
+                                   int row_stride, int lane) {
+  const float* row = partials + (long)r * row_stride;
+  float s = 0.f;
+  for (int p0 = 0; p0 < fb; p0 += 64) {
+    const int v = p0 + lane < fb ? __float_as_int(row[p0 + lane]) : 0;
+    const int n = min(64, fb - p0);
+    for (int p = 0; p < n; ++p)
+      s += __int_as_float(__builtin_amdgcn_readlane(v, p));
+  }
+  if (lane == 0) scalars[r] = s;
 }
 
 #define MLP_MAX_LAYERS 5
@@ -310,6 +324,53 @@
   uint64_t policy_seed, env_seed;
 };
 
+struct PPOIngestArgs {
+  NetArgs val, pol, old;
+  const float* obs;
+  const float* last_obs;
+  const float* actions;
+  const float* rewards;
+  const int* offsets;
+  const int* dones;
+  const float* log_std;
+  const float* old_log_std;
+  float* obs_out;
+  float* act_out;
+  float* rew_out;
+  int* off_out;
+  int* dones_out;
+  float* values_all;
+  float* old_logp;
+  float* logp_now;
+  int T, E, O, A;
+};
+
+__host__ __device__ inline long ppo_ingest_lds_floats(const int* vdims, int vl,
+                                                      const int* pdims, int pl) {
+  return net_lds_floats(3, vdims, vl) + 2 * net_lds_floats(0, pdims, pl) +
+         2 * pdims[pl];
+}
+
+struct PPOEpilogueArgs {
+  float* gate;
+  const float* kl;
+  float* kl_final;
+  float* iters_done;
+  float* iters_out;
+  float thr;
+  float* pol_step[MT_MAX_TENSORS];
+  float* val_step[MT_MAX_TENSORS];
+  int n_pol_steps, n_val_steps;
+  float val_bump;
+  const float* partials;
+  float* losses;
+  int rows, fb, row_stride;
+  const float* src[MT_MAX_TENSORS];
+  float* dst[MT_MAX_TENSORS];
+  int numel[MT_MAX_TENSORS];
+  int n_sync;
+};
+
 struct ReplayScatterArgs {
   const float* obs_full;
   const float* act_buf;
diff --git a/rl_replicas_amd/ops/hip/loss_kernels.hip b/rl_replicas_amd/ops/hip/loss_kernels.hip
--- a/rl_replicas_amd/ops/hip/loss_kernels.hip
+++ b/rl_replicas_amd/ops/hip/loss_kernels.hip
@@ -1,4 +1,5 @@
 #include "common.h"
+#include "rollout_steps.h"
 
 #define LOSS_THREADS 1024
 
@@ -174,18 +175,9 @@
 __global__ __launch_bounds__(256) void value_loss_finalize_rows(
     const float* __restrict__ partials, float* __restrict__ scalars, int rows,
     int fb, int row_stride) {
-  const int lane = threadIdx.x & 63;
   const int r = blockIdx.x * 4 + (threadIdx.x >> 6);
   if (r >= rows) return;
-  const float* row = partials + (long)r * row_stride;
-  float s = 0.f;
-  for (int p0 = 0; p0 < fb; p0 += 64) {
-    const int v = p0 + lane < fb ? __float_as_int(row[p0 + lane]) : 0;
-    const int n = min(64, fb - p0);
-    for (int p = 0; p < n; ++p)
-      s += __int_as_float(__builtin_amdgcn_readlane(v, p));
-  }
-  if (lane == 0) scalars[r] = s;
+  value_loss_row_sum(partials, scalars, r, fb, row_stride, threadIdx.x & 63);
 }
 
 __global__ __launch_bounds__(LOSS_THREADS) void gaussian_logp_kernel(
@@ -196,20 +188,11 @@
   __shared__ float s_base;
   for (int d = threadIdx.x; d < D; d += LOSS_THREADS)
     s_sigma[d] = __expf(log_std[d]);
-  if (threadIdx.x == 0) {
-    float b = 0.f;
-    for (int d = 0; d < D; ++d) b += log_std[d];
-    s_base = b + 0.5f * (float)D * LOG_2PI;
-  }
-  __syncthreads();
-  for (int r = tid; r < B; r += gridDim.x * LOSS_THREADS) {
-    float q = 0.f;
-    for (int d = 0; d < D; ++d) {
-      const float z = (actions[(long)r * D + d] - mean[(long)r * D + d]) / s_sigma[d];
-      q += z * z;
-    }
-    logp[r] = -0.5f * q - s_base;
-  }
+  if (threadIdx.x == 0) s_base = gaussian_logp_base(log_std, D);
+  __syncthreads();
+  for (int r = tid; r < B; r += gridDim.x * LOSS_THREADS)
+    logp[r] = gaussian_logp_row(actions, (long)r * D, mean, (long)r * D, s_sigma,
+                                s_base, D);
 }
 
 __global__ __launch_bounds__(LOSS_THREADS) void gaussian_kl_kernel(
diff --git a/rl_replicas_amd/ops/hip/ppo_ingest_kernels.hip b/rl_replicas_amd/ops/hip/ppo_ingest_kernels.hip
--- /dev/null
+++ b/rl_replicas_amd/ops/hip/ppo_ingest_kernels.hip
@@ -0,0 +1,78 @@
+#include "common.h"
+#include "rollout_steps.h"
+
+template <int NT>
+__global__ __launch_bounds__(NT) void ppo_ingest_rows_f32(PPOIngestArgs a) {
+  constexpr int LDSW = ROLLOUT_LDSW;
+  constexpr int ROWS = ROLLOUT_ROWS;
+  extern __shared__ float smem[];
+  float* const st = smem;
+  float* const buf0 = st + ROWS * LDSW;
+  float* const buf1 = buf0 + ROWS * LDSW;
+  float* const wl_val = buf1 + ROWS * LDSW;
+
+  const int tid = threadIdx.x;
+  const int lane = tid & 63;
+  const int wave = tid >> 6;
+  const int T = a.T, E = a.E, O = a.O, A = a.A;
+  const int row0 = blockIdx.x * ROWS;
+
+  const NetStage val = net_stage<NT, false>(a.val, wl_val, tid);
+  float* const wl_pol = val.end;
+  const NetStage pol = net_stage<NT, false>(a.pol, wl_pol, tid);
+  float* const wl_old = pol.end;
+  const NetStage old = net_stage<NT, false>(a.old, wl_old, tid);
+  float* const sigma = old.end;
+  float* const sigma_old = sigma + A;
+
+  for (int idx = tid; idx < ROWS * O; idx += NT) {
+    const int r = idx / O, c = idx % O;
+    const int row = row0 + r;
+    float v = 0.f;
+    if (row < T) {
+      v = a.obs[(long)row * O + c];
+      a.obs_out[(long)row * O + c] = v;
+    } else if (row < T + E) {
+      v = a.last_obs[(long)(row - T) * O + c];
+    }
+    st[r * LDSW + c] = v;
+  }
+  for (int idx = tid; idx < ROWS * A; idx += NT) {
+    const int row = row0 + idx / A;
+    if (row < T) a.act_out[(long)row * A + idx % A] = a.actions[(long)row * A + idx % A];
+  }
+  for (int i = blockIdx.x * NT + tid; i < T; i += gridDim.x * NT) a.rew_out[i] = a.rewards[i];
+  for (int i = blockIdx.x * NT + tid; i <= E; i += gridDim.x * NT) a.off_out[i] = a.offsets[i];
+  for (int i = blockIdx.x * NT + tid; i < E; i += gridDim.x * NT) a.dones_out[i] = a.dones[i];
+  for (int d = tid; d < A; d += NT) {
+    sigma[d] = __expf(a.log_std[d]);
+    sigma_old[d] = __expf(a.old_log_std[d]);
+  }
+  __syncthreads();
+
+  const int row = row0 + tid;
+  const bool owner = tid < ROWS;
+
+  const float* out =
+      net_forward<NT, LDSW, false>(a.val, st, buf0, buf1, wl_val, val.bl, wave, lane);
+  if (owner && row < T + E) a.values_all[row] = out[tid * LDSW];
+  __syncthreads();
+
+  out = net_forward<NT, LDSW, false>(a.pol, st, buf0, buf1, wl_pol, pol.bl, wave, lane);
+  if (owner && row < T)
+    a.logp_now[row] = gaussian_logp_row(a.actions, (long)row * A, out, tid * LDSW, sigma,
+                                        gaussian_logp_base(a.log_std, A), A);
+  __syncthreads();
+
+  out = net_forward<NT, LDSW, false>(a.old, st, buf0, buf1, wl_old, old.bl, wave, lane);
+  if (owner && row < T)
+    a.old_logp[row] = gaussian_logp_row(a.actions, (long)row * A, out, tid * LDSW,
+                                        sigma_old, gaussian_logp_base(a.old_log_std, A), A);
+}
+
+void launch_ppo_ingest_rows(const PPOIngestArgs& a, hipStream_t stream) {
+  const dim3 g((a.T + a.E + ROLLOUT_ROWS - 1) / ROLLOUT_ROWS);
+  const size_t lds = ppo_ingest_lds_floats(a.val.dims, a.val.n_layers, a.pol.dims,
+                                           a.pol.n_layers) * sizeof(float);
+  hipLaunchKernelGGL((ppo_ingest_rows_f32<256>), g, dim3(256), lds, stream, a);
+}
diff --git a/rl_replicas_amd/ops/hip/rollout_steps.h b/rl_replicas_amd/ops/hip/rollout_steps.h
--- a/rl_replicas_amd/ops/hip/rollout_steps.h
+++ b/rl_replicas_amd/ops/hip/rollout_steps.h
@@ -141,6 +141,23 @@
   for (int c = 0; c < n_cuts; ++c)
     if (cut_step[c] == t) slot = c;
   return slot;
+}
+
+DEV_INLINE float gaussian_logp_base(const float* log_std, int D) {
+  float b = 0.f;
+  for (int d = 0; d < D; ++d) b += log_std[d];
+  return b + 0.5f * (float)D * LOG_2PI;
+}
+
+DEV_INLINE float gaussian_logp_row(const float* __restrict__ actions, long aoff,
+                                   const float* __restrict__ mean, long moff,
+                                   const float* sigma, float base, int D) {
+  float q = 0.f;
+  for (int d = 0; d < D; ++d) {
+    const float z = (actions[aoff + d] - mean[moff + d]) / sigma[d];
+    q += z * z;
+  }
+  return -0.5f * q - base;
 }
 
 DEV_INLINE float uniform_sample_elem(float low, float high, uint64_t seed,
diff --git a/rl_replicas_amd/ops/hip/update_kernels.hip b/rl_replicas_amd/ops/hip/update_kernels.hip
--- a/rl_replicas_amd/ops/hip/update_kernels.hip
+++ b/rl_replicas_amd/ops/hip/update_kernels.hip
@@ -53,6 +53,44 @@
   }
 }
 
+__global__ __launch_bounds__(256) void ppo_epoch_epilogue(PPOEpilogueArgs a) {
+  const int row_blocks = (a.rows + 3) / 4;
+  const int b = blockIdx.x;
+  const int tid = threadIdx.x;
+  if (b < row_blocks) {
+    const int r = b * 4 + (tid >> 6);
+    if (r >= a.rows) return;
+    value_loss_row_sum(a.partials, a.losses, r, a.fb, a.row_stride, tid & 63);
+    return;
+  }
+  if (b == row_blocks) {
+    __shared__ float s_done;
+    if (tid == 0) {
+      if (*a.gate != 0.f) {
+        *a.kl_final = *a.kl;
+        *a.iters_done += 1.f;
+        if (*a.kl > a.thr) *a.gate = 0.f;
+      }
+      s_done = *a.iters_done;
+    }
+    __syncthreads();
+    const float done = s_done;
+    if (tid < a.n_pol_steps) a.pol_step[tid][0] += done;
+    if (tid < a.n_val_steps) a.val_step[tid][0] += a.val_bump;
+    if (tid == 0) {
+      *a.iters_out = done;
+      *a.iters_done = 0.f;
+      *a.gate = 1.f;
+    }
+    return;
+  }
+  const int t = b - row_blocks - 1;
+  if (t >= a.n_sync) return;
+  const float* s = a.src[t];
+  float* d = a.dst[t];
+  for (int i = tid; i < a.numel[t]; i += 256) d[i] = s[i];
+}
+
 __global__ __launch_bounds__(256) void fused_polyak_kernel(PolyakArgs a) {
   const int t = blockIdx.x;
   if (t >= a.n_tensors) return;
diff --git a/rl_replicas_amd/samplers/device_sampler.py b/rl_replicas_amd/samplers/device_sampler.py
--- a/rl_replicas_amd/samplers/device_sampler.py
+++ b/rl_replicas_amd/samplers/device_sampler.py
@@ -49,6 +49,7 @@
         self._bufs = None
         self._graphs: Dict[tuple, object] = {}
         self._graph_ctr: Optional[torch.Tensor] = None
+        self._episode_indices: Dict[tuple, tuple] = {}
 
     def _get_bufs(self, steps: int, obs_dim: int, act_dim: int, device):
         if self._bufs is None or self._bufs[0].shape[0] != steps:
@@ -146,6 +147,24 @@
         self._obs = obs
         return obs_buf, act_buf, rew_buf, finals
 
+    def _episode_index(self, steps: int, cuts: Tuple[int, ...]):
+        key = (steps, cuts)
+        cached = self._episode_indices.get(key)
+        if cached is None:
+            N = self.num_envs
+            seg_bounds = segment_bounds(steps, cuts)
+            offsets_np = np.zeros(N * len(seg_bounds) + 1, dtype=np.int32)
+            np.cumsum(np.tile([e - s for s, e, _ in seg_bounds], N), out=offsets_np[1:])
+            dones_np = np.tile(np.asarray([d for _, _, d in seg_bounds], dtype=np.int32), N)
+            device = self.env.device
+            if len(self._episode_indices) >= 64:
+                self._episode_indices.clear()
+            cached = self._episode_indices[key] = (
+                torch.as_tensor(offsets_np, device=device),
+                torch.as_tensor(dones_np, device=device),
+            )
+        return cached
+
     def _build_experience(self, steps: int, cuts: Tuple[int, ...], obs_buf,
                           act_buf, rew_buf, finals, obs_dim: int,
                           act_dim: int) -> Experience:
@@ -167,9 +186,8 @@
         last_obs = torch.stack(lasts, dim=1).reshape(N * n_segs, obs_dim)
 
         seg_lengths = [e - s for s, e, _ in seg_bounds]
-        offsets_np = np.zeros(N * n_segs + 1, dtype=np.int32)
-        np.cumsum(np.tile(seg_lengths, N), out=offsets_np[1:])
         dones_pattern = [d for _, _, d in seg_bounds]
+        episode_offsets, episode_dones = self._episode_index(steps, cuts)
 
         seg_returns = torch.stack(
             [rew_t[:, s:e].sum(dim=1) for s, e, _ in seg_bounds], dim=1
@@ -197,10 +215,8 @@
                 "observations": flat_obs,
                 "actions": flat_act,
                 "rewards": flat_rew,
-                "episode_offsets": torch.as_tensor(offsets_np, device=device),
-                "episode_dones": torch.as_tensor(
-                    np.tile(dones_pattern, N), device=device
-                ),
+                "episode_offsets": episode_offsets,
+                "episode_dones": episode_dones,
                 "last_observations": last_obs,
                 "next_observations": flat_next,
                 "step_dones": step_dones.reshape(-1),
diff --git a/setup.py b/setup.py
--- a/setup.py
+++ b/setup.py
@@ -18,6 +18,7 @@
         os.path.join(HIP_DIR, "env_kernels.hip"),
         os.path.join(HIP_DIR, "rollout_kernels.hip"),
         os.path.join(HIP_DIR, "rollout_fused_kernels.hip"),
+        os.path.join(HIP_DIR, "ppo_ingest_kernels.hip"),
         os.path.join(HIP_DIR, "cartpole_rollout_kernels.hip"),
         os.path.join(HIP_DIR, "pendulum_rollout_kernels.hip"),
         os.path.join(HIP_DIR, "pendulum_collect_kernels.hip"),
```

Measured after the change: 1.813 million env-steps/s, median of 6. 1.15x the previous value.
